# iacopo97/Multimodal-SAM-Adapter

Measured on AMD Instinct MI355X. Metric: images/sec encoder fwd @1024x1024 RGB+LiDAR ViT-L, higher is better.
Workload: dtype split-operand MFMA: fp16 hi + e5m2 cross terms (h8c / h8 planes, ViT / interaction / up-conv GEMMs) fp16 hi/lo pairs x3 (TwinConvNeXt: f3 planes) and bf16 hi/lo x3 (neck, head); attention blocks with the rel-pos terms fused: every contraction on one fp16 MFMA (q, k, v, P rounded to fp16) in the bloc

## Files before the change

include/mmsa.h:

```cpp
#ifndef MMSA_H
#define MMSA_H
#include <stddef.h>
#include <stdint.h>
#ifdef __cplusplus
extern "C" {
#endif

#ifdef MMSA_BUILDING_LIBRARY
typedef hipStream_t mmsa_stream_t;
#else
typedef void* mmsa_stream_t;
#endif

#include "mmsa_version.h"
int mmsa_version(void);
const char* mmsa_last_error(void);

int mmsa_debug_poison_lds(unsigned pattern, mmsa_stream_t stream);
int mmsa_event_create(void** ev);
int mmsa_event_record(void* ev, mmsa_stream_t stream);
int mmsa_event_elapsed_ms(void* start, void* stop, float* ms);
int mmsa_event_destroy(void* ev);

enum { MMSA_ACT_NONE = 0, MMSA_ACT_GELU = 1, MMSA_ACT_RELU = 2, MMSA_ACT_RELU6 = 3, MMSA_ACT_HSWISH = 4, MMSA_ACT_SIGMOID = 5 };

enum { MMSA_DT_F32 = 0, MMSA_DT_F16 = 1, MMSA_DT_F64 = 2 };

enum { MMSA_FMT_B3 = 0, MMSA_FMT_H8 = 1, MMSA_FMT_H8C = 2, MMSA_FMT_F3 = 3, MMSA_FMT_W8 = 4  };

int mmsa_ms_deform_attn_forward(const void* value, const int64_t* spatial_shapes, const int64_t* level_start_index,
                                const void* sampling_loc, const void* attn_weight, void* out, int batch,
                                int spatial_size, int num_heads, int channels, int num_levels, int num_query,
                                int num_point, int im2col_step, int dtype, mmsa_stream_t stream);

int mmsa_ms_deform_attn_backward(const void* value, const int64_t* spatial_shapes, const int64_t* level_start_index,
                                 const void* sampling_loc, const void* attn_weight, const void* grad_output,
                                 void* grad_value, void* grad_sampling_loc, void* grad_attn_weight, int batch,
                                 int spatial_size, int num_heads, int channels, int num_levels, int num_query,
                                 int num_point, int im2col_step, int dtype, mmsa_stream_t stream);

int mmsa_msda_fused(const float* value, const int64_t* spatial_shapes, const int64_t* level_start_index,
                    const float* raw, long ldraw, const float* ref_points, float* out, long ldo,
                    uint16_t* out_planes, long ldop , int out_fmt , int batch,
                    int spatial_size, int num_heads, int channels, int num_levels, int num_query, int num_point,
                    float* clamp_max , mmsa_stream_t stream);

int mmsa_msda_fused_planes(const uint16_t* value_planes, long ldvp, int lo_bytes, const int64_t* spatial_shapes, const int64_t* level_start_index,
                           const float* raw, long ldraw, const float* ref_points, float* out, long ldo,
                           uint16_t* out_planes, long ldop, int out_fmt, int batch,
                           int spatial_size, int num_heads, int channels, int num_levels, int num_query, int num_point,
                           float* clamp_max, mmsa_stream_t stream);

int mmsa_rowstats_finalize(const float* rowstats, int rows, int strips, int D, float eps, float* mean_rstd, mmsa_stream_t stream);

int mmsa_zero_bytes(void* p, size_t bytes, mmsa_stream_t stream);
int mmsa_gemm_split3(const float* A, const uint16_t* Ap, long lda, long strideA,
                     const uint16_t* Wp, long strideW,
                     const float* bias, long strideBias, const float* colscale, const float* resid, long ldr,
                     long strideR, int resid_mod, float beta, float* C, long ldc, long strideC,
                     uint16_t* Cp, long ldcp, long strideCp, int M, int N, int K,
                     int batch, int act, float alpha, int out_mode, int ps_H, int ps_W, int ps_C, int fmt, int cp_fmt,
// ... 122 lines not shown
```

include/mmsa_version.h:

```cpp
#ifndef MMSA_VERSION_H
#define MMSA_VERSION_H
#define MMSA_ABI_VERSION 106
#endif
```

multimodal-sam-adapter_amd/csrc/attention.hip:

```cpp
#include "common.h"

typedef __attribute__((ext_vector_type(4))) short s16x4;
#define LDS_AS __attribute__((address_space(3)))

struct AttnArgs {
  const float* qkv; long ldq;
  const float* qkv_bias;
  const unsigned short* qp;
  const unsigned short* bp;
  unsigned short* op;
  int ofmt;
  int vf;
  const float* rp;
  const unsigned short* relg;
  float* out; long ldo;
  int B, H, W, heads, D;
  int ws;
  int nWw;
  int Nk;
  int KH, KW;
  int KHs, KWs;
  unsigned magicKW;
  float scale;
  float* guard;
};

template <int HD, bool PL, bool FB, bool REL = false, int VF = 0>
__global__ __launch_bounds__(256, (FB && HD <= 64) ? 2 : 1) void attn_kernel(AttnArgs a) {
  static_assert(VF == 0 || PL, "the fp16 paths read planes");
  static_assert(VF != 2 || REL, "the all-fp16 form exists for the fused rel-pos kernel");
  constexpr int NCH = HD / 8;
  constexpr int KS = HD / 32;
  constexpr int DT = HD / 16;
  constexpr int VSTR = 2 * HD + 32;
  constexpr int KPL = NCH * 64 * 16;
  constexpr int VPL = 64 * VSTR;
  extern __shared__ __attribute__((aligned(16))) unsigned char smem[];
  unsigned char* Khi = smem;
  unsigned char* Klo = Khi + KPL;
  unsigned char* Vhi = Klo + KPL;
  unsigned char* Vlo = Vhi + VPL;
  float* bh = reinterpret_cast<float*>(Vlo + VPL);
  float* bw = bh + 128 * a.KHs;

  const int tid = threadIdx.x, lane = tid & 63, wave = tid >> 6;
  const int l15 = lane & 15, G = lane >> 4;
  const unsigned wg_ = mmsa_xcd_order(mmsa_block_lin(), mmsa_block_count());
  const int bx_ = (int)(wg_ % gridDim.x);
  const int head = (int)((wg_ / gridDim.x) % gridDim.y), b = (int)(wg_ / (gridDim.x * gridDim.y));
  const int T = a.H * a.W;
  const int nqb = (a.Nk + 127) / 128;
  const int grp = bx_ / nqb;
  const int q0 = (bx_ % nqb) * 128;
  const int wi = a.ws ? grp / a.nWw : 0, wj = a.ws ? grp % a.nWw : 0;

  auto token_of = [&](int j) -> int {
    if (j >= a.Nk) return -2;
    if (a.ws == 0) return j;
    const int r = j / a.ws, c = j - r * a.ws;
    const int hh = wi * a.ws + r, ww = wj * a.ws + c;
    return (hh < a.H && ww < a.W) ? hh * a.W + ww : -1;
  };
// ... 21 lines not shown
      for (int u = 0; u < 4; ++u) {
        const int i = i0 + 256 * u;
        if (i < total4) {
          const int ql = i / nf4, c4 = i - ql * nf4;
          float* d = bh + ql * a.KHs + 4 * c4;
          d[0] = v[u].x; d[1] = v[u].y; d[2] = v[u].z; d[3] = v[u].w;
        }
      }
    }
  } else {
    const int ncol = a.KH + a.KW;
    const float* rpb = a.rp + ((long)b * a.heads + head) * T * ncol;
    for (int i = tid; i < 128 * ncol; i += 256) {
      const int ql = i / ncol, cidx = i - ql * ncol;
      const int tq = token_of(q0 + ql);
      const float v = tq >= 0 ? rpb[(long)tq * ncol + cidx] : 0.f;
      if (cidx < a.KH) bh[ql * a.KHs + cidx] = v;
      else bw[ql * a.KWs + (cidx - a.KH)] = v;
    }
  }

  bf16x8 qh[2][KS], ql_[2][KS];
  int tq_sub[2];
#pragma unroll
  for (int sub = 0; sub < 2; ++sub) {
    const int jq = q0 + wave * 32 + sub * 16 + l15;
    const int tq = token_of(jq);
    tq_sub[sub] = tq;
    const long qrow = (long)(tq >= 0 ? tq : 0) * a.ldq;
    const float* qp = qkv_b + qrow;
#pragma unroll
    for (int ks = 0; ks < KS; ++ks) {
      if constexpr (PL) {
        const unsigned short* qq = pq_b + qrow + ilv(colq + ks * 32 + 8 * G);
        qh[sub][ks] = *reinterpret_cast<const bf16x8*>(qq);
        if constexpr (VF != 2) ql_[sub][ks] = *reinterpret_cast<const bf16x8*>(qq + 32);
        continue;
      }
      float4 v0 = *reinterpret_cast<const float4*>(qp + ks * 32 + 8 * G);
      float4 v1 = *reinterpret_cast<const float4*>(qp + ks * 32 + 8 * G + 4);
      v0.x *= a.scale; v0.y *= a.scale; v0.z *= a.scale; v0.w *= a.scale;
      v1.x *= a.scale; v1.y *= a.scale; v1.z *= a.scale; v1.w *= a.scale;
      uint2 h0, l0, h1, l1;
      f3_split4(v0, h0, l0);
      f3_split4(v1, h1, l1);
      uint4 hh4 = make_uint4(h0.x, h0.y, h1.x, h1.y), ll4 = make_uint4(l0.x, l0.y, l1.x, l1.y);
      qh[sub][ks] = __builtin_bit_cast(bf16x8, hh4);
      ql_[sub][ks] = __builtin_bit_cast(bf16x8, ll4);
    }
  }

  float bwr[2][4][4];
  if constexpr (REL) {
    float* bwt = reinterpret_cast<float*>(smem);
    int qc[2][2];
#pragma unroll
    for (int sub = 0; sub < 2; ++sub) {
      const int tok = min(q0 + wave * 32 + sub * 16 + l15, a.Nk - 1);
      qc[sub][0] = tok / a.W;
      qc[sub][1] = tok - qc[sub][0] * a.W;
    }
#pragma unroll
    for (int ax = 0; ax < 2; ++ax) {
      const int Kx = ax ? a.KW : a.KH;
      float* tab = ax ? bwt : bh;
      const int tstr = ax ? a.KWs : a.KHs;
#pragma unroll 2
// ... 38 lines not shown
  } else if constexpr (FB) {
    const float* rpb = a.rp + ((long)b * a.heads + head) * T * (a.KH + a.KW) + a.KH;
#pragma unroll
    for (int sub = 0; sub < 2; ++sub) {
      const int tq = tq_sub[sub];
#pragma unroll
      for (int t = 0; t < 4; ++t) {
        float4 v = make_float4(0.f, 0.f, 0.f, 0.f);
        if (tq >= 0) v = *reinterpret_cast<const float4*>(rpb + (long)tq * (a.KH + a.KW) + 16 * t + 4 * G);
        bwr[sub][t][0] = v.x * 1.4426950408889634f;
        bwr[sub][t][1] = v.y * 1.4426950408889634f;
        bwr[sub][t][2] = v.z * 1.4426950408889634f;
        bwr[sub][t][3] = v.w * 1.4426950408889634f;
      }
    }
  }

  constexpr int NF4 = HD / 16;
  constexpr int NU = HD / 32;
  const int skey = (tid & 7) + 8 * (tid >> 5), squart = (tid >> 3) & 3;
  float4 rk[NF4], rv[NF4];
  uint4 rkh[NU], rkl[NU], rvh[NU], rvl[NU];
  unsigned kv_keep = 0xffffffffu;
  auto and4 = [](uint4 v, unsigned m) { return make_uint4(v.x & m, v.y & m, v.z & m, v.w & m); };
#define LOAD_KV(kb_)                                                                         \
  do {                                                                                       \
    const int tk_ = token_of((kb_) * 64 + skey);                                             \
    if constexpr (PL) {                                                                      \
                                                  \
      const unsigned short* rowp_ = tk_ >= 0 ? pq_b + (long)tk_ * a.ldq : a.bp;                                                \
      const unsigned keep_ = tk_ == -2 ? 0u : 0xffffffffu;                                                                     \
      _Pragma("unroll") for (int i = 0; i < NU; ++i) {                                       \
        const int c = squart * (HD / 4) + 8 * i;                                             \
        const unsigned short* kr_ = rowp_ + ilv(colk + c);                                   \
        const unsigned short* vr_ = rowp_ + ilv(colv + c);                                   \
        rkh[i] = *reinterpret_cast<const uint4*>(kr_);                                       \
        if constexpr (VF != 2) rkl[i] = *reinterpret_cast<const uint4*>(kr_ + 32);           \
        rvh[i] = *reinterpret_cast<const uint4*>(vr_);                                       \
        if constexpr (VF == 0) rvl[i] = *reinterpret_cast<const uint4*>(vr_ + 32);           \
      }                                                                                      \
      kv_keep = keep_;                                                                       \
    } else {                                                                                 \
      _Pragma("unroll") for (int i = 0; i < NF4; ++i) {                                      \
        const int c = squart * (HD / 4) + 4 * i;                                             \
        if (tk_ >= 0) {                                                                      \
          const float* p = qkv_b + (long)tk_ * a.ldq + c;                                    \
          rk[i] = *reinterpret_cast<const float4*>(p + a.D);                                 \
          rv[i] = *reinterpret_cast<const float4*>(p + 2 * a.D);                             \
        } else if (tk_ == -1) {                                                              \
          rk[i] = *reinterpret_cast<const float4*>(kbias + c);                               \
          rv[i] = *reinterpret_cast<const float4*>(vbias + c);                               \
        } else {                                                                             \
          rk[i] = make_float4(0.f, 0.f, 0.f, 0.f);                                           \
          rv[i] = rk[i];                                                                     \
        }                                                                                    \
      }                                                                                      \
    }                                                                                        \
  } while (0)
#define STORE_KV(Kh_, Kl_, Vh_, Vl_)                                                                           \
  do {                                                                                       \
    if constexpr (PL) {                                                                      \
      _Pragma("unroll") for (int i = 0; i < NU; ++i) {                                       \
        const int c = squart * (HD / 4) + 8 * i;                                             \
        const int ko = (c >> 3) * (64 * 16) + skey * 16;                                     \
        *reinterpret_cast<uint4*>((Kh_) + ko) = and4(rkh[i], kv_keep);                         \
        if constexpr (VF != 2) *reinterpret_cast<uint4*>((Kl_) + ko) = and4(rkl[i], kv_keep);  \
        const int vo = skey * VSTR + c * 2;                                                  \
        *reinterpret_cast<uint4*>((Vh_) + vo) = and4(rvh[i], kv_keep);                         \
// ... 187 lines not shown
  }

  if (a.guard) {
    const float gv = wave_max(amax) * 0.6931471805599453f;
    if (lane == 0 && gv > *reinterpret_cast<volatile float*>(a.guard)) atomicMax(reinterpret_cast<unsigned*>(a.guard), __float_as_uint(gv));
  }
#pragma unroll
  for (int sub = 0; sub < 2; ++sub) {
    float l = l_run[sub];
    l += __shfl_xor(l, 16, 64);
    l += __shfl_xor(l, 32, 64);
    const float inv = 1.0f / l;
    const int tq = tq_sub[sub];
    if constexpr (PL) {
      const long orow = (long)b * T + (tq >= 0 ? tq : 0);
#pragma unroll
      for (int d = 0; d < DT; ++d)
        store_planes8_pair_any<16>(a.op, a.ldo, orow, MMSA_PAD64(a.D), head * HD + 16 * d + 8 * (G >> 1),
                                   make_float4(o[sub][d][0] * inv, o[sub][d][1] * inv, o[sub][d][2] * inv, o[sub][d][3] * inv), a.ofmt, G & 1, tq >= 0);
    } else if (tq >= 0) {
      const long oo = ((long)b * T + tq) * a.ldo + head * HD + 4 * G;
#pragma unroll
      for (int d = 0; d < DT; ++d)
        *reinterpret_cast<float4*>(a.out + oo + 16 * d) = make_float4(o[sub][d][0] * inv, o[sub][d][1] * inv, o[sub][d][2] * inv, o[sub][d][3] * inv);
    }
  }
}

static int attention_launch(AttnArgs a, int B, int H, int W, int heads, int head_dim, int window_size, float scale,
                            bool planes, hipStream_t stream) {
  MMSA_CHECK_ARG(B > 0 && H > 0 && W > 0 && heads > 0 && window_size >= 0, "attention: bad shape");
  MMSA_CHECK_ARG(head_dim == 64 || head_dim == 32 || head_dim == 96, "attention: head_dim %d not supported (32, 64 or 96; other widths are zero-padded per head by the caller, e.g. ViT-H's 80 -> 96)", head_dim);
  const int D = heads * head_dim;
  MMSA_CHECK_ARG(a.ldq >= (planes ? 6L : 3L) * D && (a.ldq & 7) == 0 && a.ldo >= (planes ? (a.ofmt == MMSA_FMT_H8C ? 3L * MMSA_PAD64(D) : 2L * D) : 1L * D) && (a.ldo & 3) == 0,
                 "attention: bad leading dimensions");
  a.B = B; a.H = H; a.W = W; a.heads = heads; a.D = D; a.ws = window_size; a.scale = scale;
  int ngroups;
  if (window_size > 0) {
    a.nWw = cdiv(W, window_size);
    ngroups = cdiv(H, window_size) * a.nWw;
    a.Nk = window_size * window_size;
    a.KH = a.KW = window_size;
  } else {
    a.nWw = 1;
    ngroups = 1;
    a.Nk = H * W;
    a.KH = H;
    a.KW = W;
  }
  a.KHs = a.KH | 1;
  a.KWs = a.KW | 1;
  a.magicKW = (unsigned)(((1u << 24) + a.KW - 1) / a.KW);
  for (int j = 0; j < a.Nk; ++j) {
    if ((int)(((unsigned long long)(unsigned)j * a.magicKW) >> 24) != j / a.KW || (unsigned long long)j * a.magicKW >= (1ull << 32)) {
      mmsa_set_error("attention: key grid too large for the in-kernel index arithmetic (Nk=%d KW=%d)", a.Nk, a.KW);
      return MMSA_ERR_ARG;
    }
  }
  const int VSTR = 2 * head_dim + 32;
  const bool fb = window_size == 0 && W == 64 && (H % 4) == 0;
  const size_t smem = 2 * (head_dim / 8) * 64 * 16 + 2 * 64 * VSTR + (size_t)128 * (a.KHs + (fb ? 0 : a.KWs)) * sizeof(float);
  MMSA_CHECK_ARG(smem <= 160 * 1024, "attention: bias tables do not fit LDS (KH=%d KW=%d)", a.KH, a.KW);
  dim3 grid(ngroups * cdiv(a.Nk, 128), heads, B);
#define ATTN_LAUNCH(HD_, PL_, FB_)                                                                                         \
  do {                                                                                                                     \
    if (smem > 64 * 1024) (void)hipFuncSetAttribute((const void*)attn_kernel<HD_, PL_, FB_>, hipFuncAttributeMaxDynamicSharedMemorySize, (int)smem); \
    hipLaunchKernelGGL((attn_kernel<HD_, PL_, FB_>), grid, dim3(256), smem, stream, a);                                    \
  } while (0)
#define ATTN_LAUNCH_VF(HD_, FB_)                                                                                           \
  do {                                                                                                                     \
    if (smem > 64 * 1024) (void)hipFuncSetAttribute((const void*)attn_kernel<HD_, true, FB_, false, 1>, hipFuncAttributeMaxDynamicSharedMemorySize, (int)smem); \
    hipLaunchKernelGGL((attn_kernel<HD_, true, FB_, false, 1>), grid, dim3(256), smem, stream, a);                      \
  } while (0)
  MMSA_CHECK_ARG(a.vf == 0 || (planes && a.vf == (a.relg ? 2 : 1)), "attention: v_fmt %d (0 = bf16 hi/lo planes; 1 = h8 planes for the v columns, the entry with a rel-pos prepass; 2 = h8 planes throughout, the fused rel-pos entry)", a.vf);
  if (head_dim == 64) {
    if (planes && a.relg) {
      MMSA_CHECK_ARG(fb && H <= 64 && 128 * a.KWs * (int)sizeof(float) <= 2 * 8 * 64 * 16 + 2 * 64 * VSTR, "attention: the fused rel-pos path needs a W = 64, H <= 64 global grid");
      if (a.vf) hipLaunchKernelGGL((attn_kernel<64, true, true, true, 2>), grid, dim3(256), smem, stream, a);
      else hipLaunchKernelGGL((attn_kernel<64, true, true, true>), grid, dim3(256), smem, stream, a);
    } else if (planes && a.vf) { if (fb) ATTN_LAUNCH_VF(64, true); else ATTN_LAUNCH_VF(64, false); }
    else if (planes) { if (fb) ATTN_LAUNCH(64, true, true); else ATTN_LAUNCH(64, true, false); }
    else { if (fb) ATTN_LAUNCH(64, false, true); else ATTN_LAUNCH(64, false, false); }
  } else if (head_dim == 96) {
    if (planes && a.vf) { if (fb) ATTN_LAUNCH_VF(96, true); else ATTN_LAUNCH_VF(96, false); }
    else if (planes) { if (fb) ATTN_LAUNCH(96, true, true); else ATTN_LAUNCH(96, true, false); }
    else { if (fb) ATTN_LAUNCH(96, false, true); else ATTN_LAUNCH(96, false, false); }
  } else {
    if (planes && a.vf) { if (fb) ATTN_LAUNCH_VF(32, true); else ATTN_LAUNCH_VF(32, false); }
    else if (planes) { if (fb) ATTN_LAUNCH(32, true, true); else ATTN_LAUNCH(32, true, false); }
    else { if (fb) ATTN_LAUNCH(32, false, true); else ATTN_LAUNCH(32, false, false); }
  }
#undef ATTN_LAUNCH_VF
#undef ATTN_LAUNCH
  MMSA_CHECK_LAUNCH("attention");
  return MMSA_OK;
}

extern "C" int mmsa_attention(const float* qkv, long ldq, const float* qkv_bias, const float* rp, float* out, long ldo,
                              int B, int H, int W, int heads, int head_dim, int window_size, float scale,
                              hipStream_t stream) {
  MMSA_CHECK_ARG(qkv && qkv_bias && rp && out, "attention: null pointer");
  MMSA_CHECK_ARG(((((uintptr_t)qkv) | ((uintptr_t)out) | ((uintptr_t)qkv_bias)) & 15) == 0, "attention: pointers must be 16-byte aligned");
  AttnArgs a = {};
  a.qkv = qkv; a.ldq = ldq; a.qkv_bias = qkv_bias; a.rp = rp; a.out = out; a.ldo = ldo;
  return attention_launch(a, B, H, W, heads, head_dim, window_size, scale, false, stream);
}

extern "C" int mmsa_attention_planes(const unsigned short* qkv_p, long ldq, const unsigned short* bias_p, const float* rp,
                                     unsigned short* out_p, long ldo, int B, int H, int W,
                                     int heads, int head_dim, int window_size, float scale, int out_fmt, int v_fmt, float* max_abs_logit,
                                     hipStream_t stream) {
// ... 120 lines not shown
```

multimodal-sam-adapter_amd/csrc/common.h:

```cpp
#pragma once
#include <hip/hip_runtime.h>
#include <stdint.h>
#include <stdio.h>
#include <stdarg.h>

#define MMSA_OK 0
#define MMSA_ERR_ARG (-1)
#define MMSA_ERR_LAUNCH (-2)

#define MMSA_BUILDING_LIBRARY 1
#include "../../include/mmsa.h"
void mmsa_set_error(const char* fmt, ...);

#ifdef MMSA_DEBUG_KNOBS
#include <stdlib.h>
static inline int mmsa_knob_env(const char* name, int dflt) { const char* v = getenv(name); return v ? atoi(v) : dflt; }
#define MMSA_KNOB(name_, dflt_) mmsa_knob_env(name_, dflt_)
#else
#define MMSA_KNOB(name_, dflt_) (dflt_)
#endif

#define MMSA_CHECK_ARG(cond, ...)            \
  do {                                       \
    if (!(cond)) {                           \
// ... 104 lines not shown
__device__ __forceinline__ void f3_split2(float a, float b, unsigned& hi, unsigned& lo) {
  a = __builtin_amdgcn_fmed3f(a, -MMSA_F3_MAX, MMSA_F3_MAX);
  b = __builtin_amdgcn_fmed3f(b, -MMSA_F3_MAX, MMSA_F3_MAX);
  split2_f16(a, b, hi, lo);
}
__device__ __forceinline__ void f3_split4(const float4 v, uint2& hi, uint2& lo) {
  f3_split2(v.x, v.y, hi.x, lo.x);
  f3_split2(v.z, v.w, hi.y, lo.y);
}
__device__ __forceinline__ void split4_fmt(const float4 v, uint2& hi, uint2& lo, int fmt) {
  if (fmt == MMSA_FMT_F3) f3_split4(v, hi, lo);
  else split4(v, hi, lo);
}

template <bool UPPER, bool COMP = false>
__device__ __forceinline__ void h8_split2(float a, float b, unsigned& hi, unsigned& lo8, unsigned& qh8) {
  a = __builtin_amdgcn_fmed3f(a, -MMSA_H8_MAX, MMSA_H8_MAX);
  b = __builtin_amdgcn_fmed3f(b, -MMSA_H8_MAX, MMSA_H8_MAX);
  const mmsa_f32x2 v = {a, b};
  const mmsa_h2 h = __builtin_convertvector(v, mmsa_h2);
  const mmsa_f32x2 hf = __builtin_convertvector(h, mmsa_f32x2);
  constexpr float ls_ = COMP ? MMSA_H8_LO_SCALE * MMSA_H8C_LO_COMP : MMSA_H8_LO_SCALE;
  const mmsa_f32x2 l = (v - hf) * ls_;
  hi = __builtin_bit_cast(unsigned, h);
  lo8 = (unsigned)__builtin_amdgcn_cvt_pk_bf8_f32(l.x, l.y, (int)lo8, UPPER);
  qh8 = (unsigned)__builtin_amdgcn_cvt_pk_bf8_f32(hf.x, hf.y, (int)qh8, UPPER);
}
template <bool COMP = false>
__device__ __forceinline__ void h8_split4(const float4 v, uint2& hi, unsigned& lo8, unsigned& qh8) {
  lo8 = 0u; qh8 = 0u;
  h8_split2<false, COMP>(v.x, v.y, hi.x, lo8, qh8);
  h8_split2<true, COMP>(v.z, v.w, hi.y, lo8, qh8);
}
__host__ __device__ __forceinline__ int h8_lo_off(int c) { return ((c >> 5) << 7) + 64 + (((c & 31) >> 3) << 4) + (c & 7); }

__device__ __forceinline__ void store_planes4(unsigned short* row, int c, const float4 v, int fmt) {
  if (fmt == MMSA_FMT_H8) {
    uint2 hi; unsigned lo8, qh8;
    h8_split4(v, hi, lo8, qh8);
    *reinterpret_cast<uint2*>(row + ilv(c)) = hi;
    unsigned char* rb = reinterpret_cast<unsigned char*>(row) + h8_lo_off(c);
    *reinterpret_cast<unsigned*>(rb) = lo8;
    *reinterpret_cast<unsigned*>(rb + 8) = qh8;
  } else {
    uint2 hh, ll;
    split4_fmt(v, hh, ll, fmt);
    *reinterpret_cast<uint2*>(row + ilv(c)) = hh;
    *reinterpret_cast<uint2*>(row + ilv(c) + 32) = ll;
  }
}

template <int XOR>
__device__ __forceinline__ void store_planes8_pair(unsigned short* row, int c8, const float4 v, int fmt, bool odd, bool do_store) {
  uint2 mine_hi, mine_x;
  if (fmt == MMSA_FMT_H8) h8_split4(v, mine_hi, mine_x.x, mine_x.y);
  else split4_fmt(v, mine_hi, mine_x, fmt);
  const uint2 snd = odd ? mine_hi : mine_x;
  uint2 rcv;
  rcv.x = __shfl_xor(snd.x, XOR, 64);
  rcv.y = __shfl_xor(snd.y, XOR, 64);
  uint4 pk;
  if (!odd) pk = make_uint4(mine_hi.x, mine_hi.y, rcv.x, rcv.y);
  else if (fmt == MMSA_FMT_H8) pk = make_uint4(rcv.x, mine_x.x, rcv.y, mine_x.y);
  else pk = make_uint4(rcv.x, rcv.y, mine_x.x, mine_x.y);
  const int off = odd ? (fmt == MMSA_FMT_H8 ? h8_lo_off(c8) >> 1 : ilv(c8) + 32) : ilv(c8);
  if (do_store) *reinterpret_cast<uint4*>(row + off) = pk;
// ... 170 lines not shown
```

multimodal-sam-adapter_amd/csrc/gemm_epilogue_regs.inc:

```
#ifndef MMSA_EPI_REGS
#define MMSA_EPI_REGS 1
#endif
#ifndef MMSA_EPI_REGS_FP32
#define MMSA_EPI_REGS_FP32 0
#endif
#ifndef MMSA_EPI_ROWS
#define MMSA_EPI_ROWS 1
#endif
#ifndef MMSA_EPI_NOSTORE
#define MMSA_EPI_NOSTORE 0
#endif
#if MMSA_EPI_NOSTORE
#define EPI_ST16(ptr_, val_) { const uint4 v__ = __builtin_bit_cast(uint4, val_); asm volatile("" :: "v"(v__.x), "v"(v__.y), "v"(v__.z), "v"(v__.w), "v"(ptr_)); }
#else
#define EPI_ST16(ptr_, val_) { *reinterpret_cast<uint4*>(ptr_) = __builtin_bit_cast(uint4, val_); }
#endif
#ifndef EPI_STAMP
#define EPI_STAMP(i_)
#define EPI_STAMP_WAIT()
#define EPI_STAMP_DEFAULTED_ 1
#endif
      bool regs_done = false;
      if constexpr (MMSA_EPI_REGS && EPI_UNROLL && !GEN && (ACT == ACT_NONE || ACT == ACT_GELU)) {
        const bool interior_ = m0 + V2_BM <= a.M && n0 + a.bn <= a.N;
        const bool al16_ = ((((uintptr_t)bias) | ((uintptr_t)colscale) | ((uintptr_t)resid) | ((uintptr_t)C) | ((uintptr_t)Cp) | ((uintptr_t)a.rn_cs)) & 15) == 0 &&
                           ((a.ldc | a.ldr) & 3) == 0 && (a.ldcp & 7) == 0 && (a.strideBias & 3) == 0;
        if (interior_ && al16_ && V2_DBG(a) == 0 && !cp_split && (ni4 || (C && !Cp && !a.rs_out && !a.rn_mr))) {
          auto swap16_ = [](unsigned& x_, unsigned& y_) {
            const auto r_ = __builtin_amdgcn_permlane16_swap(x_, y_, false, false);
            x_ = r_[0]; y_ = r_[1];
          };
          auto epi_regs_ = [&](auto c_C, auto c_R, auto c_CPF, auto c_RS, auto c_RN, auto c_CS) {
// ... 13 lines not shown
              }
              if constexpr (kRN) sn_[ni] = *reinterpret_cast<const float4*>(a.rn_cs + (long)bz * a.strideBias + ci);
            }
            float2 mr_[4];
            if constexpr (kRN) {
#pragma unroll
              for (int mi = 0; mi < 4; ++mi) mr_[mi] = *reinterpret_cast<const float2*>(a.rn_mr + 2 * ((long)bz * a.M + row0 + 16 * mi));
            }
#ifndef MMSA_EPI_PREFETCH_ALL
#define MMSA_EPI_PREFETCH_ALL 0
#endif
            float4 rra[4][4];
            const float* rbase = nullptr;
            if constexpr (kR) {
              rbase = resid + (long)row0 * a.ldr + col0;
#pragma unroll
              for (int mi = 0; mi < (MMSA_EPI_PREFETCH_ALL ? 4 : 1); ++mi)
#pragma unroll
                for (int ni = 0; ni < 4; ++ni) rra[mi][ni] = *reinterpret_cast<const float4*>(rbase + (long)mi * 16 * a.ldr + ni * 16);
            }
            EPI_STAMP(1) EPI_STAMP_WAIT() EPI_STAMP(2)
            float* cbase = nullptr;
            if constexpr (kC) cbase = C + (long)row0 * a.ldc + col0;
            const int hcol = 16 * (g & 1) + 8 * (g >> 1);
            const int schunk = 16 * (2 * (g & 1) + (g >> 1));
            unsigned short* prow = nullptr;
            unsigned char* plo = nullptr;
            long pstep = 0;
            if constexpr (kCPF == MMSA_FMT_H8C) {
              unsigned short* pb = Cp + (long)(row0 >> 1) * a.ldcp;
              prow = pb + (row0 & 1) * cp_kpad + nb_ + hcol;
              plo = reinterpret_cast<unsigned char*>(pb + 2 * cp_kpad) + (row0 & 1) * 64 + ((nb_ >> 6) << 7) + schunk;
              pstep = 8 * a.ldcp;
            } else if constexpr (kCPF >= 0) {
              prow = Cp + (long)row0 * a.ldcp + ((nb_ >> 5) << 6) + hcol;
              pstep = 16 * a.ldcp;
            }
            unsigned long long cwm_ = 0ull;
            constexpr bool kWatch = MMSA_CLAMP_WATCH && MMSA_CW_REGS && (kCPF == MMSA_FMT_H8C || kCPF == MMSA_FMT_H8 || kCPF == MMSA_FMT_F3);
            constexpr float kLimit = (kCPF == MMSA_FMT_F3) ? MMSA_F3_MAX : MMSA_H8_MAX;
            float* rsb = nullptr;
            if constexpr (kRS) rsb = a.rs_out + (((long)bz * a.M + row0) * a.rs_strips + (nb_ >> 6)) * 2;
#pragma unroll
            for (int mi = 0; mi < 4; ++mi) {
              if constexpr (kR && !MMSA_EPI_PREFETCH_ALL) {
                if (mi < 3) {
#pragma unroll
                  for (int ni = 0; ni < 4; ++ni) rra[mi + 1][ni] = *reinterpret_cast<const float4*>(rbase + (long)(mi + 1) * 16 * a.ldr + ni * 16);
                }
              }
              float s1 = 0.f, s2 = 0.f;
              uint2 H[4], Lp[4];
              unsigned L8[4], Q8[4];
#pragma unroll
              for (int ni = 0; ni < 4; ++ni) {
                float4 o;
                if constexpr (kRN) {
                  const float mu = mr_[mi].x, rs = mr_[mi].y;
                  o = make_float4(fmaf(rs, fmaf(-mu, sn_[ni].x, acc[ni][mi][0]), bn_[ni].x), fmaf(rs, fmaf(-mu, sn_[ni].y, acc[ni][mi][1]), bn_[ni].y),
                                  fmaf(rs, fmaf(-mu, sn_[ni].z, acc[ni][mi][2]), bn_[ni].z), fmaf(rs, fmaf(-mu, sn_[ni].w, acc[ni][mi][3]), bn_[ni].w));
                } else {
                  o = make_float4(acc[ni][mi][0] + bn_[ni].x, acc[ni][mi][1] + bn_[ni].y, acc[ni][mi][2] + bn_[ni].z, acc[ni][mi][3] + bn_[ni].w);
                }
                acc[ni][mi] = (f32x4){0.f, 0.f, 0.f, 0.f};
                if constexpr (ACT == ACT_GELU) o = gelu4(o);
                if constexpr (kCS) { o.x *= cn_[ni].x; o.y *= cn_[ni].y; o.z *= cn_[ni].z; o.w *= cn_[ni].w; }
                if constexpr (kR) { o.x += a.beta * rra[mi][ni].x; o.y += a.beta * rra[mi][ni].y; o.z += a.beta * rra[mi][ni].z; o.w += a.beta * rra[mi][ni].w; }
                if constexpr (kC) EPI_ST16(cbase + (long)mi * 16 * a.ldc + ni * 16, o)
                if constexpr (kRS) {
                  s1 += (o.x + o.y) + (o.z + o.w);
                  s2 += fmaf(o.x, o.x, o.y * o.y) + fmaf(o.z, o.z, o.w * o.w);
                }
                if constexpr (kWatch) cwm_ |= __builtin_amdgcn_ballot_w64(fmaxf(fmaxf(fabsf(o.x), fabsf(o.y)), fmaxf(fabsf(o.z), fabsf(o.w))) > kLimit);
                if constexpr (kCPF == MMSA_FMT_H8C) h8_split4<true>(o, H[ni], L8[ni], Q8[ni]);
                else if constexpr (kCPF == MMSA_FMT_H8) h8_split4<false>(o, H[ni], L8[ni], Q8[ni]);
                else if constexpr (kCPF == MMSA_FMT_F3) f3_split4(o, H[ni], Lp[ni]);
                else if constexpr (kCPF == MMSA_FMT_B3) split4(o, H[ni], Lp[ni]);
              }
              if constexpr (kCPF >= 0) {
                unsigned short* pr = prow + (long)mi * pstep;
#pragma unroll
                for (int p = 0; p < 2; ++p) {
                  swap16_(H[2 * p].x, H[2 * p + 1].x);
                  swap16_(H[2 * p].y, H[2 * p + 1].y);
                  const uint4 hv = make_uint4(H[2 * p].x, H[2 * p].y, H[2 * p + 1].x, H[2 * p + 1].y);
                  if constexpr (kCPF == MMSA_FMT_H8C) {
                    EPI_ST16(pr + 32 * p, hv)
                  } else {
                    EPI_ST16(pr + 64 * p, hv)
                    if constexpr (kCPF == MMSA_FMT_H8) {
                      swap16_(L8[2 * p], L8[2 * p + 1]);
                      swap16_(Q8[2 * p], Q8[2 * p + 1]);
                      EPI_ST16(reinterpret_cast<unsigned char*>(pr + 64 * p - hcol) + 64 + schunk, make_uint4(L8[2 * p], L8[2 * p + 1], Q8[2 * p], Q8[2 * p + 1]))
                    } else {
                      swap16_(Lp[2 * p].x, Lp[2 * p + 1].x);
                      swap16_(Lp[2 * p].y, Lp[2 * p + 1].y);
                      EPI_ST16(pr + 64 * p + 32, make_uint4(Lp[2 * p].x, Lp[2 * p].y, Lp[2 * p + 1].x, Lp[2 * p + 1].y))
                    }
                  }
                }
                if constexpr (kCPF == MMSA_FMT_H8C) {
                  swap16_(L8[0], L8[1]);
                  swap16_(L8[2], L8[3]);
                  EPI_ST16(plo + (long)mi * pstep * 2, make_uint4(L8[0], L8[1], L8[2], L8[3]))
                }
              }
              if constexpr (kRS) {
                {
                  const auto r1 = __builtin_amdgcn_permlane32_swap(__float_as_uint(s1), __float_as_uint(s1), false, false);
                  const auto r2 = __builtin_amdgcn_permlane32_swap(__float_as_uint(s2), __float_as_uint(s2), false, false);
                  s1 = __uint_as_float(r1[0]) + __uint_as_float(r1[1]);
                  s2 = __uint_as_float(r2[0]) + __uint_as_float(r2[1]);
                }
                {
                  const auto r1 = __builtin_amdgcn_permlane16_swap(__float_as_uint(s1), __float_as_uint(s1), false, false);
                  const auto r2 = __builtin_amdgcn_permlane16_swap(__float_as_uint(s2), __float_as_uint(s2), false, false);
                  s1 = __uint_as_float(r1[0]) + __uint_as_float(r1[1]);
                  s2 = __uint_as_float(r2[0]) + __uint_as_float(r2[1]);
                }
// ... 40 lines not shown
#pragma unroll
                  for (int i = 0; i < 4; ++i) rq[(mi + 1) & 1][i] = *reinterpret_cast<const float4*>(rb_ + (long)(16 * (mi + 1) + 4 * i) * a.ldr);
                }
              }
#pragma unroll
              for (int ni = 0; ni < 4; ++ni) {
                *reinterpret_cast<f32x4*>(stg_ + l15 * 68 + ni * 16 + 4 * g) = acc[ni][mi];
                acc[ni][mi] = (f32x4){0.f, 0.f, 0.f, 0.f};
              }
#pragma unroll
              for (int i = 0; i < 4; ++i) {
                const float4 t = *reinterpret_cast<const float4*>(stg_ + (rl + 4 * i) * 68 + cl4);
                float4 o;
                if constexpr (kRN) {
                  const float mu = mr4[mi][i].x, rs = mr4[mi][i].y;
                  o = make_float4(fmaf(rs, fmaf(-mu, sn4.x, t.x), bv4.x), fmaf(rs, fmaf(-mu, sn4.y, t.y), bv4.y), fmaf(rs, fmaf(-mu, sn4.z, t.z), bv4.z), fmaf(rs, fmaf(-mu, sn4.w, t.w), bv4.w));
                } else {
                  o = make_float4(t.x + bv4.x, t.y + bv4.y, t.z + bv4.z, t.w + bv4.w);
                }
                if constexpr (kCS) { o.x *= cv4.x; o.y *= cv4.y; o.z *= cv4.z; o.w *= cv4.w; }
                if constexpr (kR) { const float4 r_ = rq[mi & 1][i]; o.x += a.beta * r_.x; o.y += a.beta * r_.y; o.z += a.beta * r_.z; o.w += a.beta * r_.w; }
                EPI_ST16(cb_ + (long)(16 * mi + 4 * i) * a.ldc, o)
              }
              EPI_STAMP(3 + mi)
            }
          };
          const int cpf_ = Cp ? cp_base : -1;
          const bool rn_ = a.rn_mr != nullptr, rso_ = a.rs_out != nullptr;
          const bool scaled_ = colscale != nullptr || a.alpha != 1.0f;
#define EPI_REGS_RUN1(C_, R_, F_, S_, N_, CS_)                                                                                        \
  { epi_regs_(std::integral_constant<bool, C_>{}, std::integral_constant<bool, R_>{}, std::integral_constant<int, F_>{},               \
              std::integral_constant<bool, S_>{}, std::integral_constant<bool, N_>{}, std::integral_constant<bool, CS_>{}); regs_done = true; }
#define EPI_REGS_RUN(C_, R_, F_, S_, N_) { if (!scaled_) EPI_REGS_RUN1(C_, R_, F_, S_, N_, false) }
          if (!C && !resid && !rso_) {
            if (cpf_ == MMSA_FMT_H8C) { if (rn_) EPI_REGS_RUN(false, false, MMSA_FMT_H8C, false, true) else EPI_REGS_RUN(false, false, MMSA_FMT_H8C, false, false) }
            else if (cpf_ == MMSA_FMT_H8) { if (rn_) EPI_REGS_RUN(false, false, MMSA_FMT_H8, false, true) else EPI_REGS_RUN(false, false, MMSA_FMT_H8, false, false) }
            else if (cpf_ == MMSA_FMT_F3 && !rn_) EPI_REGS_RUN(false, false, MMSA_FMT_F3, false, false)
            else if (cpf_ == MMSA_FMT_B3 && !rn_) EPI_REGS_RUN(false, false, MMSA_FMT_B3, false, false)
          } else if (C && cpf_ < 0 && !rso_ && MMSA_EPI_ROWS) {
            if constexpr (ACT == ACT_NONE) {
              if (scaled_) {
                if (!rn_) { if (resid) epi_rows_(std::true_type{}, std::false_type{}, std::true_type{}); else epi_rows_(std::false_type{}, std::false_type{}, std::true_type{}); regs_done = true; }
              } else if (resid) { if (!rn_) { epi_rows_(std::true_type{}, std::false_type{}, std::false_type{}); regs_done = true; } }
              else if (rn_) { epi_rows_(std::false_type{}, std::true_type{}, std::false_type{}); regs_done = true; }
              else { epi_rows_(std::false_type{}, std::false_type{}, std::false_type{}); regs_done = true; }
            }
          } else if (C && !rn_) {
            if constexpr (ACT == ACT_NONE) {
              if (resid && rso_ && cpf_ == MMSA_FMT_H8C) { if (scaled_) EPI_REGS_RUN1(true, true, MMSA_FMT_H8C, true, false, true) else EPI_REGS_RUN1(true, true, MMSA_FMT_H8C, true, false, false) }
              else if (resid && rso_ && cpf_ == MMSA_FMT_F3) EPI_REGS_RUN(true, true, MMSA_FMT_F3, true, false)
              else if (MMSA_EPI_REGS_FP32 && resid && !rso_ && cpf_ < 0) EPI_REGS_RUN(true, true, -1, false, false)
              else if (MMSA_EPI_REGS_FP32 && !resid && !rso_ && cpf_ < 0) EPI_REGS_RUN(true, false, -1, false, false)
            }
          }
#undef EPI_REGS_RUN
#undef EPI_REGS_RUN1
#undef EPI_ST16
        }
      }
```

multimodal-sam-adapter_amd/csrc/gemm_h8c.hip:

```cpp
#include "common.h"
#include "gemm_h8c_shared.h"

#define HC_H_UNIT 49152
#define HC_L_UNIT 24576
#define HC_LDS_H(i_) ((i_) * HC_H_UNIT)
#define HC_LDS_L(i_) (2 * HC_H_UNIT + (i_) * (HC_L_UNIT + 16384))
#define HC_LDS_TOTAL (2 * HC_H_UNIT + 2 * HC_L_UNIT + 16384)

#ifdef HC_EPI_STAMP
__device__ unsigned long long g_hc_estamps[8 * 16];
extern "C" int mmsa_debug_epi_stamps(unsigned long long* host_out) { return (int)hipMemcpyFromSymbol(host_out, HIP_SYMBOL(g_hc_estamps), sizeof(g_hc_estamps)); }
#define EPI_STAMP(i_) { if (estamp_on_) { __builtin_amdgcn_sched_barrier(0); et_[i_] = __builtin_readcyclecounter(); __builtin_amdgcn_sched_barrier(0); } }
#define EPI_STAMP_WAIT() { if (estamp_on_) asm volatile("s_waitcnt vmcnt(0)" ::: "memory"); }
#else
#define EPI_STAMP(i_)
#define EPI_STAMP_WAIT()
#endif
template <bool GEN, int ACT>
__global__ __launch_bounds__(512, 1) void gemm_h8c_kernel(GemmV2Args a) {
  constexpr bool PP = true;
  constexpr bool EPI_UNROLL = ACT >= 0;
  constexpr int V2_BM = 256;
  constexpr int V2_NST = 3;
  extern __shared__ __attribute__((aligned(16))) unsigned char smem[];
  const int tid = threadIdx.x, lane = tid & 63;
  const int wave = __builtin_amdgcn_readfirstlane(tid >> 6);
  const int wm = wave >> 1, wn = wave & 1, grp = wave >> 2;
  const int l15 = lane & 15, g = lane >> 4;
  const int K = a.K;
  const int np = K >> 6;
  const bool ni4 = true;
  const int swid = 64;
  const int G = gridDim.x;
  int rb = blockIdx.x;
  V2_XCD_REMAP(rb, G)
  const int my_tiles = (a.ntiles - rb + G - 1) / G;
  if (my_tiles <= 0) return;
  V2_SLACK_STAGGER(a, rb, G)
  const int total = my_tiles * np;

  H8C_DMA_LANE();
  const int lds_ha = wave * 32 * 128, lds_hw = 32768 + wave * 16 * 128;
  const int lds_la = wave * 2048, lds_lw = 16384 + wave * 1024;
  const unsigned ldaB = (unsigned)(a.lda * 2), ldwB = (unsigned)(a.ldw * 2);
  const unsigned K2 = (unsigned)K * 2u, K4 = (unsigned)K * 4u;
  H8C_A_LANE_HI();
  const unsigned LW_E = (unsigned)(drow >> 1) * ldwB + (unsigned)(drow & 1) * K2 + dpiece, LW_O = LW_E ^ 64u;
  H8C_A_LANE_LO();
  const unsigned LLW = (unsigned)drow * ldwB + K4 + lq;

  const unsigned char *hA, *hW, *lA, *lW;
  int h_m0 = 0, h_n0 = 0, l_m0 = 0, l_n0 = 0;
// ... 106 lines not shown
    H8C_SB();                                                                                                         \
     \
     \
    if (FAST_) { ++lp_j; ++lp_p; ++hp_j; ++hp_p; } else { if (do_l) HC_L_ADVANCE() if (do_h) HC_H_ADVANCE() }          \
    H8C_SB();                                                                                                         \
    if (FAST_) H8C_WAIT(9); else if (tail || last) H8C_WAIT(0); else if (!skipw) H8C_WAIT(9);                         \
    H8C_BAR()                                                                                                         \
    if (!(FAST_)) nowait = 0;                                                                                         \
    ++j;                                                                                                              \
  }

  for (int tdone = 0; tdone < my_tiles; ++tdone) {
    if (grp) H8C_BAR()
    bool interior;
    { int bz_, m0_, n0_; H8C_TILE(tile, 256, bz_, m0_, n0_) interior = m0_ + 256 <= a.M && n0_ + 128 <= a.N; }
    int p = 0;
    HC_PAIR(0)
    ++p;
    if (interior) {
#pragma unroll 1
      for (; p < np - 2; ++p) HC_PAIR(1)
      if (hp_p == np) { hp_p = 0; hp_tile += G; if (hp_j < total) HC_SET_H(hp_tile) }
    }
#pragma unroll 1
    for (; p < np; ++p) HC_PAIR(0)
    if (!grp) H8C_BAR()
    if (V2_DBG(a) == 2) H8C_NO_EPILOGUE() else {
#ifdef HC_EPI_STAMP
      unsigned long long et_[9] = {0, 0, 0, 0, 0, 0, 0, 0, 0};
      const bool estamp_on_ = blockIdx.x == 0 && tdone == 1;
#endif
      EPI_STAMP(0)
#define EPI_STAGING_BASE (smem + (((j - 1) & 1) ? 2 * HC_H_UNIT + HC_L_UNIT : 2 * HC_H_UNIT))
#include "gemm_v2_epilogue.inc"
      EPI_STAMP(7)
#ifdef HC_EPI_STAMP
      asm volatile("s_waitcnt lgkmcnt(0)" ::: "memory");
      H8C_BAR()
      EPI_STAMP(8)
      if (estamp_on_ && (threadIdx.x & 63) == 0) {
#pragma unroll
        for (int q_ = 0; q_ < 9; ++q_) g_hc_estamps[wave * 16 + q_] = et_[q_];
      }
#endif
    }
    asm volatile("s_waitcnt lgkmcnt(0)" ::: "memory");
    H8C_BAR()
    tile += G;
  }
}

int mmsa_gemm_h8c_dispatch(const GemmV2Args& a, int grid, bool gen, int act, hipStream_t stream) {
  static MmsaPerDevice per_dev_ = {};
  (void)mmsa_per_device(per_dev_, [] {
#define HC_ATTR(GEN_, ACT_) (void)hipFuncSetAttribute((const void*)gemm_h8c_kernel<GEN_, ACT_>, hipFuncAttributeMaxDynamicSharedMemorySize, HC_LDS_TOTAL);
    V2_EPI_TABLE(HC_ATTR)
#undef HC_ATTR
  });
#define HC_LAUNCH(GEN_, ACT_) if (v2_epi_serves(gen, act, GEN_, ACT_)) hipLaunchKernelGGL((gemm_h8c_kernel<GEN_, ACT_>), dim3(grid), dim3(512), HC_LDS_TOTAL, stream, a);
  V2_EPI_TABLE(HC_LAUNCH)
#undef HC_LAUNCH
  MMSA_CHECK_LAUNCH("gemm_split3(h8c)");
  return MMSA_OK;
}
```

multimodal-sam-adapter_amd/csrc/gemm_h8c_w8.hip:

```cpp
#include "gemm_h8c_shared.h"

typedef __attribute__((ext_vector_type(2))) _Float16 hw_h2;

#define HW_H_UNIT 40960
#define HW_L_UNIT 32768
#define HW_LDS_H(i_) ((i_) * HW_H_UNIT)
#define HW_LDS_L(i_) (2 * HW_H_UNIT + (i_) * (HW_L_UNIT + 16384))
#define HW_LDS_TOTAL (2 * HW_H_UNIT + 2 * HW_L_UNIT + 16384)

__device__ __forceinline__ uint2 w8_cvt4(unsigned c, float s) {
  const hw_h2 lo = __builtin_amdgcn_cvt_scalef32_pk_f16_fp8(c, s, false);
  const hw_h2 hi = __builtin_amdgcn_cvt_scalef32_pk_f16_fp8(c, s, true);
  return make_uint2(__builtin_bit_cast(unsigned, lo), __builtin_bit_cast(unsigned, hi));
}

template <bool GEN, int ACT>
__global__ __launch_bounds__(512, 1) void gemm_h8c_w8_kernel(GemmV2Args a) {
  constexpr bool PP = true;
  constexpr bool EPI_UNROLL = ACT >= 0;
  constexpr int V2_BM = 256;
  constexpr int V2_NST = 3;
  extern __shared__ __attribute__((aligned(16))) unsigned char smem[];
  const int tid = threadIdx.x, lane = tid & 63;
  const int wave = __builtin_amdgcn_readfirstlane(tid >> 6);
  const int wm = wave >> 1, wn = wave & 1, grp = wave >> 2;
  const int l15 = lane & 15, g = lane >> 4;
  const int K = a.K;
  const int np = K >> 6;
  const bool ni4 = true;
  const int swid = 64;
  const int G = gridDim.x;
  int rb = blockIdx.x;
  V2_XCD_REMAP(rb, G)
  const int my_tiles = (a.ntiles - rb + G - 1) / G;
  if (my_tiles <= 0) return;
  V2_SLACK_STAGGER(a, rb, G)
  const int total = my_tiles * np;
  const int nsteps = np >> 1, total_s = my_tiles * nsteps;

  H8C_DMA_LANE();
  const int lds_ha = wave * 32 * 128, lds_hw = 32768 + wave * 1024;
  const int lds_la = wave * 2048;
  const unsigned ldaB = (unsigned)(a.lda * 2);
  const unsigned ldwB = (unsigned)(a.ldw * 2);
  const unsigned K2 = (unsigned)K * 2u, K4 = (unsigned)K * 4u;
  H8C_A_LANE_HI();
  const int wcol = lane >> 2;
  const unsigned wpiece = (unsigned)(((lane & 3) ^ ((lane >> 4) & 3)) * 16);
  const unsigned LW = (unsigned)wcol * ldwB + wpiece;
  H8C_A_LANE_LO();
// ... 143 lines not shown
    H8C_SB();                                                                                                         \
    if (tail || last) H8C_WAIT(0); else if ((FAST_) || !skipw) { if (ODD_) H8C_WAIT(5); else H8C_WAIT(9); }          \
    H8C_BAR()                                                                                                         \
    if (!(FAST_)) nowait = 0;                                                                                         \
    ++j;                                                                                                              \
  }

  for (int tdone = 0; tdone < my_tiles; ++tdone) {
    if (grp) H8C_BAR()
    bool interior;
    { int bz_, m0_, n0_; H8C_TILE(tile, 256, bz_, m0_, n0_) interior = m0_ + 256 <= a.M && n0_ + 128 <= a.N; }
    HW_SCALES(tile)
    int p = 0;
    HW_PAIR(0, 0)
    ++p;
    HW_PAIR(0, 1)
    ++p;
    if (interior) {
#pragma unroll 1
      for (; p < np - 2; p += 2) { HW_PAIR(1, 0) HW_PAIR(1, 1) }
      if (hp_p == np) { hp_p = 0; hp_tile += G; if (hp_j < total) HW_SET_H(hp_tile) }
      if (lp_p == nsteps) { lp_p = 0; lp_tile += G; if (lp_j < total_s) HW_SET_L(lp_tile) }
    }
#pragma unroll 1
    for (; p < np; ) {
      HW_PAIR(0, 0)
      ++p;
      HW_PAIR(0, 1)
      ++p;
    }
    if (!grp) H8C_BAR()
    if (V2_DBG(a) == 2) H8C_NO_EPILOGUE() else {
#define EPI_STAGING_BASE (smem + ((((j - 1) >> 1) & 1) ? HW_LDS_L(1) - 16384 : HW_LDS_L(0)))
#include "gemm_v2_epilogue.inc"
    }
    asm volatile("s_waitcnt lgkmcnt(0)" ::: "memory");
    H8C_BAR()
    tile += G;
  }
}

int mmsa_gemm_h8c_w8_dispatch(const GemmV2Args& a, int grid, bool gen, int act, hipStream_t stream) {
  static MmsaPerDevice per_dev_ = {};
  (void)mmsa_per_device(per_dev_, [] {
#define HW_ATTR(GEN_, ACT_) (void)hipFuncSetAttribute((const void*)gemm_h8c_w8_kernel<GEN_, ACT_>, hipFuncAttributeMaxDynamicSharedMemorySize, HW_LDS_TOTAL);
    V2_EPI_TABLE(HW_ATTR)
#undef HW_ATTR
  });
#define HW_LAUNCH(GEN_, ACT_) if (v2_epi_serves(gen, act, GEN_, ACT_)) hipLaunchKernelGGL((gemm_h8c_w8_kernel<GEN_, ACT_>), dim3(grid), dim3(512), HW_LDS_TOTAL, stream, a);
  V2_EPI_TABLE(HW_LAUNCH)
#undef HW_LAUNCH
  MMSA_CHECK_LAUNCH("gemm_split3(h8c x w8)");
  return MMSA_OK;
}
```

multimodal-sam-adapter_amd/csrc/gemm_split3.hip:

```cpp
#include "common.h"

struct GemmArgs {
  const float* A; const unsigned short* Ap; long lda; long strideA;
  const unsigned short* Wp; long strideW;
  const float* bias; long strideBias;
  const float* colscale;
  const float* resid; long ldr; long strideR; int resid_mod; float beta;
  float* C; long ldc; long strideC;
  unsigned short* Cp; long ldcp; long strideCp;
  int M, N, K;
  int act; float alpha;
  int out_mode; int ps_H, ps_W, ps_C;
  int cp_fmt;
  float* clamp_max;
};

#define BM 128
#define BN 128
#define BK 32
#define PLANE_BYTES (4 * 128 * 16)
#define STAGE_BYTES (4 * PLANE_BYTES)

template <bool AP, bool GEN, bool F16 = false>
__global__ __launch_bounds__(256) void gemm_split3_kernel(GemmArgs a) {
// ... 253 lines not shown
#pragma unroll
  for (int j = 0; j < 8; ++j) acc[j] = wave_sum(acc[j]);
  if (lane < 8 && n0 + lane < a.N) {
    const int n = n0 + lane;
    float v = acc[0];
#pragma unroll
    for (int j = 1; j < 8; ++j) v = lane == j ? acc[j] : v;
    if (a.bias) v += a.bias[(long)bz * a.strideBias + n];
    v = apply_act(v, a.act) * (a.colscale ? a.colscale[(long)bz * a.strideBias + n] * a.alpha : a.alpha);
    if (a.resid) v += a.beta * a.resid[(long)bz * a.strideR + (long)m * a.ldr + n];
    a.C[(long)bz * a.strideC + (long)m * a.ldc + n] = v;
  }
}


extern "C" int mmsa_gemm_split3(const float* A, const unsigned short* Ap, long lda, long strideA,
                                const unsigned short* Wp, long strideW,
                                const float* bias, long strideBias, const float* colscale,
                                const float* resid, long ldr, long strideR, int resid_mod, float beta,
                                float* C, long ldc, long strideC,
                                unsigned short* Cp, long ldcp, long strideCp,
                                int M, int N, int K, int batch, int act, float alpha,
                                int out_mode, int ps_H, int ps_W, int ps_C, int fmt, int cp_fmt, int max_grid,
                                float* rowstats_out, const float* rownorm_mean_rstd, const float* rownorm_colsum, int flavour,
                                float* clamp_max, hipStream_t stream) {
  const bool ap = Ap != nullptr;
  float* const rs_out = rowstats_out;
  const float* const rn_mr = rownorm_mean_rstd;
  const float* const rn_cs = rownorm_colsum;
  MMSA_CHECK_ARG(!rn_mr == !rn_cs, "gemm_split3: mean/rstd rows and column sums go together");
  MMSA_CHECK_ARG(!(rs_out && rn_mr), "gemm_split3: a GEMM either writes row statistics or normalises by them");
  const bool extras = rs_out || rn_mr;
  MMSA_CHECK_ARG(!extras || (ap && M >= 128), "gemm_split3: row statistics / row normalisation need activation planes and M >= 128");
  MMSA_CHECK_ARG(fmt >= MMSA_FMT_B3 && fmt <= MMSA_FMT_W8 && cp_fmt >= 0 && MMSA_CP_BASE(cp_fmt) >= MMSA_FMT_B3 && MMSA_CP_BASE(cp_fmt) <= MMSA_FMT_F3, "gemm_split3: bad plane format %d / %d", fmt, cp_fmt);
  MMSA_CHECK_ARG(MMSA_CP_SPLIT(cp_fmt) == 0 || (out_mode == 0 && MMSA_CP_SPLIT(cp_fmt) < N && MMSA_CP_BASE(cp_fmt) != MMSA_FMT_H8C), "gemm_split3: the output-format split %d needs a plain [M, N] bf16 hi/lo planes output with N=%d beyond it", MMSA_CP_SPLIT(cp_fmt), N);
  MMSA_CHECK_ARG(fmt == MMSA_FMT_B3 || fmt == MMSA_FMT_F3 || (ap && K % 64 == 0), "gemm_split3: h8 / h8c operands need A planes and K %% 64 == 0 (K=%d)", K);
  MMSA_CHECK_ARG(fmt != MMSA_FMT_F3 || ap || !Cp, "gemm_split3: f3 weights with an fp32 A write fp32 outputs only");
  MMSA_CHECK_ARG(fmt != MMSA_FMT_W8 || (K % 128 == 0 && batch == 1), "gemm_split3: W8 weights need h8c A planes, K %% 128 == 0 and one batch (K=%d, batch=%d)", K, batch);
  const bool h8c = fmt == MMSA_FMT_H8C || fmt == MMSA_FMT_W8, cp_h8c = MMSA_CP_BASE(cp_fmt) == MMSA_FMT_H8C;
  MMSA_CHECK_ARG((A || Ap) && Wp && (C || Cp), "gemm_split3: null pointer");
  MMSA_CHECK_ARG(!(A && Ap), "gemm_split3: pass either fp32 A or A planes, not both");
  MMSA_CHECK_ARG(M > 0 && N > 0 && K > 0 && batch > 0, "gemm_split3: bad shape M=%d N=%d K=%d batch=%d", M, N, K, batch);
  MMSA_CHECK_ARG(K % BK == 0, "gemm_split3: K=%d must be a multiple of %d (producers pad)", K, BK);
  if (ap) {
    MMSA_CHECK_ARG((lda & 63) == 0 && (strideA & 63) == 0 && (((uintptr_t)Ap) & 127) == 0,
                   "gemm_split3: A planes must be 128-byte aligned with lda%%64==0 (lda=%ld)", lda);
    MMSA_CHECK_ARG(lda >= (h8c ? 3L : 2L) * K, "gemm_split3: planes lda=%ld < %d*K=%d (h8c: lda is the row-PAIR stride)", lda, h8c ? 3 : 2, K);
  } else {
    MMSA_CHECK_ARG((lda & 3) == 0 && (strideA & 3) == 0 && (((uintptr_t)A) & 15) == 0, "gemm_split3: A must be 16-byte aligned with lda%%4==0 (lda=%ld)", lda);
  }
  MMSA_CHECK_ARG(lda >= K, "gemm_split3: lda=%ld < K=%d", lda, K);
  MMSA_CHECK_ARG((((uintptr_t)Wp) & 127) == 0 && (strideW & 63) == 0, "gemm_split3: weight planes must be 128-byte aligned");
  MMSA_CHECK_ARG((!C || (((uintptr_t)C) & 15) == 0) && (!resid || (((uintptr_t)resid) & 15) == 0), "gemm_split3: C/resid must be 16-byte aligned");
  MMSA_CHECK_ARG(!Cp || ((((uintptr_t)Cp) & 127) == 0 && (ldcp & 63) == 0 && (strideCp & 63) == 0), "gemm_split3: output planes must be 128-byte aligned, ldcp%%64==0");
  MMSA_CHECK_ARG(act >= ACT_NONE && act <= ACT_SIGMOID, "gemm_split3: bad act %d", act);
  if (out_mode == 1) {
    MMSA_CHECK_ARG(ps_H > 0 && ps_W > 0 && ps_C > 0 && N == 4 * ps_C && M % (ps_H * ps_W) == 0 && (ps_C & 3) == 0,
                   "gemm_split3: pixel-shuffle store needs N==4*C, M%%(H*W)==0");
    MMSA_CHECK_ARG((!C || ldc >= ps_C) && (!Cp || ldcp >= (cp_h8c ? 3L * MMSA_PAD64(ps_C) : 2L * ps_C)), "gemm_split3: ldc < C");
  } else {
    MMSA_CHECK_ARG(out_mode == 0, "gemm_split3: bad out_mode %d", out_mode);
    MMSA_CHECK_ARG((!C || ldc >= N) && (!Cp || ldcp >= (cp_h8c ? 3L * MMSA_PAD64(N) : 2L * ((N + 31) / 32 * 32))), "gemm_split3: ldc=%ld < N=%d", ldc, N);
  }
  GemmArgs a;
  a.A = A; a.Ap = Ap; a.lda = lda; a.strideA = strideA;
  a.Wp = Wp; a.strideW = strideW;
  a.bias = bias; a.strideBias = strideBias; a.colscale = colscale;
  a.resid = resid; a.ldr = ldr; a.strideR = strideR; a.resid_mod = resid_mod; a.beta = beta;
  a.C = C; a.ldc = C ? ldc : 0; a.strideC = strideC;
  a.Cp = Cp; a.ldcp = Cp ? ldcp : 0; a.strideCp = strideCp;
  a.M = M; a.N = N; a.K = K; a.act = act; a.alpha = alpha;
  a.out_mode = out_mode; a.ps_H = ps_H; a.ps_W = ps_W; a.ps_C = ps_C; a.cp_fmt = cp_fmt;
  a.clamp_max = clamp_max;
  const bool force_v1 = MMSA_KNOB("MMSA_GEMM_V1", 0) != 0;
  const bool narrow = false;
  const bool no_tiny = MMSA_KNOB("MMSA_GEMM_NO_TINY", 0) != 0;
  if (!ap && !Cp && out_mode == 0 && resid_mod <= 0 && (N <= 64 || K <= 64) && M <= 16384 && !no_tiny && !extras && fmt == MMSA_FMT_B3) {
    const int ncg = cdiv(N, 8);
    hipLaunchKernelGGL(gemm_tiny_kernel, dim3(cdiv((long)M * ncg, 4), batch), dim3(256), 0, stream, a, ncg);
    MMSA_CHECK_LAUNCH("gemm_split3(tiny)");
    return MMSA_OK;
  }
  if (ap && (fmt != MMSA_FMT_B3 || (M >= 128 && !force_v1 && !narrow))) {
    return mmsa_gemm_v2_launch(Ap, lda, strideA, Wp, strideW, bias, strideBias, colscale, resid, ldr, strideR,
                               resid_mod, beta, C, ldc, strideC, Cp, ldcp, strideCp, M, N, K, batch, act, alpha,
                               out_mode, ps_H, ps_W, ps_C, fmt, cp_fmt, max_grid, stream, rs_out, rn_mr, rn_cs, flavour, clamp_max);
  }
  MMSA_CHECK_ARG(!extras, "gemm_split3: this shape is not routed to the LDS-DMA kernel, which alone writes row statistics / normalises rows");
  MMSA_CHECK_ARG(!cp_h8c, "gemm_split3: h8c output planes are written by the LDS-DMA kernel only (activation planes in, M >= 128)");
  dim3 grid(cdiv(N, BN), cdiv(M, BM), batch);
  const bool gen = out_mode != 0 || resid_mod > 0;
  if (ap) {
    if (gen) hipLaunchKernelGGL((gemm_split3_kernel<true, true>), grid, dim3(256), 2 * STAGE_BYTES, stream, a);
    else hipLaunchKernelGGL((gemm_split3_kernel<true, false>), grid, dim3(256), 2 * STAGE_BYTES, stream, a);
  } else if (fmt == MMSA_FMT_F3) {
// ... 55 lines not shown
```

multimodal-sam-adapter_amd/csrc/gemm_v2.hip:

```cpp
#include "common.h"
#include "gemm_v2_shared.h"
template <bool GEN, int ACT, bool PP, int NW, int FMT>
__global__ __launch_bounds__(NW * 64, NW == 4 ? 2 : 1) void gemm_v2_kernel(GemmV2Args a) {
  static_assert(NW == 8 || (NW == 4 && !PP), "4-wave workgroups run the in-phase main loop");
  static_assert(FMT == MMSA_FMT_B3 || (PP && NW == 8), "the h8 and f3 operand formats run on the ping-pong kernel");
  constexpr bool EPI_UNROLL = ACT >= 0;
  constexpr int V2_BM = NW * 32;
  constexpr int V2_A_BYTES = V2_BM * 128;
  constexpr int V2_STAGE = V2_A_BYTES + V2_W_BYTES;
  constexpr int V2_NST = NW == 8 ? 3 : 2;
  constexpr int WROWS = V2_BN / NW;
  constexpr int NDMA = 4 + WROWS / 8;
  extern __shared__ __attribute__((aligned(16))) unsigned char smem[];
  const int tid = threadIdx.x;
  const int lane = tid & 63;
  const int wave = __builtin_amdgcn_readfirstlane(tid >> 6);
  const int wm = wave >> 1, wn = wave & 1;
  const int grp = wave >> 2;
  const int l15 = lane & 15, g = lane >> 4;
  const int K = a.K;
  const int nk = K / V2_BK;

  const int G = gridDim.x;
  int rb = blockIdx.x;
  V2_XCD_REMAP(rb, G)
  const int my_tiles = (a.ntiles - rb + G - 1) / G;
  if (my_tiles <= 0) return;
  V2_SLACK_STAGGER(a, rb, G)
  CLK_SAMPLE(0)
  const int total = my_tiles * nk;

  const int drow = lane >> 3;
  const int dpiece = ((lane & 7) ^ (drow >> 1)) * 8;
  const int lds_a = wave * 32 * 128;
  const int lds_w = wave * WROWS * 128;
  const unsigned char *gA, *gW;
// ... 362 lines not shown
#undef MXPAR
        }
      } else {
#define MXPAR 0
#pragma unroll 1
        for (int kt = 0; kt < kt_a; ++kt) K_STEP_PP()
        if (ni4) {
#pragma unroll 1
          for (int kt = kt_a; kt < kt_b; ++kt) K_STEP_PP_FAST(true)
        } else {
#pragma unroll 1
          for (int kt = kt_a; kt < kt_b; ++kt) K_STEP_PP_FAST(false)
        }
        if (fast_ok) {
          pf_kt = 0;
          pf_tile += G;
          if (pf_j < total) SET_TILE_SRC(pf_tile);
        }
#pragma unroll 1
        for (int kt = kt_b; kt < nk; ++kt) K_STEP_PP()
#undef MXPAR
      }
      if (!grp) __builtin_amdgcn_s_barrier();
    } else {
#define MXPAR 0
#pragma unroll 1
      for (int kt = 0; kt < nk; ++kt) K_STEP()
#undef MXPAR
    }
    const int st_cur = st == 0 ? V2_NST - 1 : st - 1;

    if (V2_DBG(a) == 2 || V2_DBG(a) == 5 || V2_DBG(a) >= 64) { tile += G; continue; }
#define EPI_STAGING_BASE (smem + st_cur * V2_STAGE)
#include "gemm_v2_epilogue.inc"
    if constexpr (PP) {
      asm volatile("s_waitcnt lgkmcnt(0)" ::: "memory");
      __builtin_amdgcn_s_barrier();
    }
    tile += G;
  }
  CLK_SAMPLE(2)
#undef K_STEP
#undef K_STEP_PP
#undef K_STEP_PP_FAST
#undef PP_WAIT
#undef PP_PIECE
#undef MFMA_CHUNK
#undef MFMA_FP8_ALL
}

int mmsa_gemm_h8c_dispatch(const GemmV2Args& a, int grid, bool gen, int act, hipStream_t stream);
int mmsa_gemm_h8c_w8_dispatch(const GemmV2Args& a, int grid, bool gen, int act, hipStream_t stream);
int mmsa_gemm_stream_try(const unsigned short* Ap, long lda, const unsigned short* Wp, const float* bias, const float* colscale, const float* resid, long ldr, float beta,
                         float* C, long ldc, unsigned short* Cp, long ldcp, int M, int N, int K, int batch, int act, float alpha, int out_mode, int resid_mod,
                         int fmt, int cp_fmt, int max_grid, const float* rs_out, const float* rn_mr, int flavour, float* clamp_max, hipStream_t stream);
int mmsa_gemm_h8c4_dispatch(const GemmV2Args& a, int grid, hipStream_t stream);

int mmsa_gemm_v2_launch(const unsigned short* Ap, long lda, long strideA,
                        const unsigned short* Wp, long strideW,
                        const float* bias, long strideBias, const float* colscale,
                        const float* resid, long ldr, long strideR, int resid_mod, float beta,
                        float* C, long ldc, long strideC,
                        unsigned short* Cp, long ldcp, long strideCp,
                        int M, int N, int K, int batch, int act, float alpha,
                        int out_mode, int ps_H, int ps_W, int ps_C, int fmt, int cp_fmt, int max_grid, hipStream_t stream,
                        float* rs_out, const float* rn_mr, const float* rn_cs, int flavour, float* clamp_max) {
// ... 9 lines not shown
  MMSA_CHECK_ARG(!rn_mr || (rn_cs && !resid && out_mode == 0 && resid_mod <= 0 && (N & 127) == 0 && ((((uintptr_t)bias) | ((uintptr_t)colscale) | ((uintptr_t)rn_cs)) & 15) == 0 && (strideBias & 3) == 0 &&
                            ((Cp && !C && (act == ACT_NONE || act == ACT_GELU || act == ACT_RELU)) ||
                             (C && !Cp && act == ACT_NONE && (M & 255) == 0 && !colscale && alpha == 1.0f && (ldc & 3) == 0 && (((uintptr_t)C) & 15) == 0))),
                 "gemm(v2): the row-normalising epilogue needs N %% 128 == 0 (N=%d), 16-byte aligned column vectors and either a planes-only output or a plain fp32 output with M %% 256 == 0 (M=%d), no activation / scale", N, M);
  a.rs_out = rs_out; a.rs_strips = N >> 6; a.rn_mr = rn_mr; a.rn_cs = rn_cs;
  a.Ap = Ap; a.lda = lda; a.strideA = strideA;
  a.Wp = Wp; a.strideW = strideW;
  const bool w8 = fmt == MMSA_FMT_W8;
  const bool h8c = fmt == MMSA_FMT_H8C || w8;
  MMSA_CHECK_ARG(!w8 || ((K & 127) == 0 && batch == 1), "gemm(v2): W8 weights need K %% 128 == 0 and one batch (K=%d, batch=%d)", K, batch);
  a.ldw = w8 ? K / 2 : h8c ? 3L * K : 2L * K;
  a.bias = bias; a.strideBias = strideBias; a.colscale = colscale;
  a.resid = resid; a.ldr = ldr; a.strideR = strideR; a.resid_mod = resid_mod; a.beta = beta;
  a.C = C; a.ldc = C ? ldc : 0; a.strideC = strideC;
  a.Cp = Cp; a.ldcp = Cp ? ldcp : 0; a.strideCp = strideCp;
  a.M = M; a.N = N; a.K = K; a.act = act; a.alpha = alpha;
  a.out_mode = out_mode; a.ps_H = ps_H; a.ps_W = ps_W; a.ps_C = ps_C;
  auto log2_exact = [](int v) { int s_ = -1; if (v > 0 && (v & (v - 1)) == 0) { s_ = 0; while ((1 << s_) < v) ++s_; } return s_; };
  a.ps_sw = log2_exact(ps_W); a.ps_sh = log2_exact(ps_H);
  a.cp_fmt = cp_fmt;
  const bool h8 = fmt == MMSA_FMT_H8 || h8c;
  MMSA_CHECK_ARG(!h8 || (K & 63) == 0, "gemm(v2): h8 operands need K %% 64 == 0 (K=%d)", K);
  MMSA_CHECK_ARG(flavour == 0 || flavour == 4 || flavour == 8, "gemm(v2): flavour %d (0 = by shape, 4, 8)", flavour);
  static MmsaPerDevice per_dev_ = {};
  const int num_cus = mmsa_per_device(per_dev_, [] {
#define V2_ATTR(GEN_, ACT_)                                                                                                   \
  (void)hipFuncSetAttribute((const void*)gemm_v2_kernel<GEN_, ACT_, false, 8, MMSA_FMT_B3>, hipFuncAttributeMaxDynamicSharedMemorySize, V2_LDS_BYTES(8)); \
  (void)hipFuncSetAttribute((const void*)gemm_v2_kernel<GEN_, ACT_, true, 8, MMSA_FMT_B3>, hipFuncAttributeMaxDynamicSharedMemorySize, V2_LDS_BYTES(8));  \
  (void)hipFuncSetAttribute((const void*)gemm_v2_kernel<GEN_, ACT_, true, 8, MMSA_FMT_H8>, hipFuncAttributeMaxDynamicSharedMemorySize, V2_LDS_BYTES(8));  \
  (void)hipFuncSetAttribute((const void*)gemm_v2_kernel<GEN_, ACT_, true, 8, MMSA_FMT_F3>, hipFuncAttributeMaxDynamicSharedMemorySize, V2_LDS_BYTES(8));  \
  (void)hipFuncSetAttribute((const void*)gemm_v2_kernel<GEN_, ACT_, false, 4, MMSA_FMT_B3>, hipFuncAttributeMaxDynamicSharedMemorySize, V2_LDS_BYTES(4));
    V2_EPI_TABLE(V2_ATTR)
#undef V2_ATTR
  });
  const int cus = (max_grid > 0 && max_grid < num_cus) ? max_grid : num_cus;
  const bool h8c4 = flavour == 4 && h8c && !w8 && out_mode == 0 && resid_mod <= 0 && act == ACT_NONE && M >= 128;
  const int nw = h8c4 ? 4 : (h8 || rs_out || rn_mr || fmt == MMSA_FMT_F3) ? 8 : flavour ? flavour : (K <= MMSA_KNOB("MMSA_GEMM_NW4_MAXK", 256) && max_grid <= 0 ? 4 : 8);
  const int bm = nw * 32, wg_per_cu = nw == 4 ? 2 : 1;
  a.nbm = cdiv(M, bm);
  a.bn = V2_BN;
  a.nbn = cdiv(N, V2_BN);
  a.ntiles = a.nbm * a.nbn * batch;
#ifdef MMSA_DEBUG_KNOBS
  a.debug = MMSA_KNOB("MMSA_GEMM_DEBUG", 0);
#endif
  if (!Cp && out_mode == 0 && resid_mod <= 0 && N >= 96 && N % 96 == 0 && !rs_out && !h8c) {
    const bool no96 = MMSA_KNOB("MMSA_GEMM_NO96", 0) != 0;
    const int nbn96 = cdiv(N, 96);
    const long t96 = (long)a.nbm * nbn96 * batch;
    const int slots = cus * wg_per_cu;
    const double c128 = (double)cdiv(a.ntiles, slots), c96 = 0.75 * (double)cdiv(t96, slots);
    if (!no96 && c96 < c128 - 1e-9) {
      a.bn = 96;
      a.nbn = nbn96;
      a.ntiles = (int)t96;
    }
  }
  const bool rowmajor = MMSA_KNOB("MMSA_GEMM_ROWMAJOR", 0) != 0;
  a.tm = a.tn = 0;
  if (!rowmajor) {
    double best = 0.0;
    for (int tn = 1; tn <= 32; tn <<= 1) {
      const int tm = 32 / tn;
      if (a.nbn % tn != 0 || a.nbm % tm != 0) continue;
      const double cost = (double)(a.nbn / tn) * M + (double)(a.nbm / tm) * N;
      if (a.tm == 0 || cost < best) { best = cost; a.tm = tm; a.tn = tn; }
    }
  }
  const int slots_ = cus * wg_per_cu;
  const int rounds_ = cdiv(a.ntiles, slots_);
  int grid = cdiv(a.ntiles, rounds_);
  a.stagger = 0;
#ifndef MMSA_GEMM_STAGGER
#define MMSA_GEMM_STAGGER 0
#endif
  if (MMSA_GEMM_STAGGER && MMSA_KNOB("MMSA_GEMM_STAGGER", 1) && nw == 8 && rounds_ >= 2 && a.ntiles % slots_ != 0) {
    grid = slots_;
    a.stagger = h8c ? (K >> 6) * 3800 + 16000 : (K >> 5) * (fmt == MMSA_FMT_H8 ? 1700 : 1900) + 16000;
  }
  const bool gen = out_mode != 0 || resid_mod > 0;
  if (w8) return mmsa_gemm_h8c_w8_dispatch(a, grid, gen, act, stream);
  if (h8c4) return mmsa_gemm_h8c4_dispatch(a, grid, stream);
  if (h8c) return mmsa_gemm_h8c_dispatch(a, grid, gen, act, stream);
  const bool pp = MMSA_KNOB("MMSA_GEMM_PP", 1) != 0;
#define V2_LAUNCH(GEN_, ACT_)                                                                                              \
  if (v2_epi_serves(gen, act, GEN_, ACT_)) {                                                                               \
    if (fmt == MMSA_FMT_H8) hipLaunchKernelGGL((gemm_v2_kernel<GEN_, ACT_, true, 8, MMSA_FMT_H8>), dim3(grid), dim3(512), V2_LDS_BYTES(8), stream, a);          \
    else if (fmt == MMSA_FMT_F3) hipLaunchKernelGGL((gemm_v2_kernel<GEN_, ACT_, true, 8, MMSA_FMT_F3>), dim3(grid), dim3(512), V2_LDS_BYTES(8), stream, a);     \
    else if (nw == 4) hipLaunchKernelGGL((gemm_v2_kernel<GEN_, ACT_, false, 4, MMSA_FMT_B3>), dim3(grid), dim3(256), V2_LDS_BYTES(4), stream, a);     \
    else if (pp) hipLaunchKernelGGL((gemm_v2_kernel<GEN_, ACT_, true, 8, MMSA_FMT_B3>), dim3(grid), dim3(512), V2_LDS_BYTES(8), stream, a);     \
    else hipLaunchKernelGGL((gemm_v2_kernel<GEN_, ACT_, false, 8, MMSA_FMT_B3>), dim3(grid), dim3(512), V2_LDS_BYTES(8), stream, a);            \
  }
  V2_EPI_TABLE(V2_LAUNCH)
#undef V2_LAUNCH
  MMSA_CHECK_LAUNCH("gemm_split3(v2)");
  return MMSA_OK;
}
```

multimodal-sam-adapter_amd/csrc/gemm_v2_epilogue.inc:

```
    {
      int lane_o_ = lane;
      asm volatile("" : "+v"(lane_o_));
      const int lane = lane_o_, l15 = lane_o_ & 15, g = lane_o_ >> 4;
    {
      const int per_b = a.nbm * a.nbn;
      const int bz = tile / per_b;
      const int rt = tile - bz * per_b;
      int tmi, tni;
      V2_TILE_MN(rt, tmi, tni);
      const int m0 = tmi * V2_BM, n0 = tni * a.bn;
      const float* bias = a.bias ? a.bias + (long)bz * a.strideBias : nullptr;
      const float* colscale = a.colscale ? a.colscale + (long)bz * a.strideBias : nullptr;
      const float* resid = a.resid ? a.resid + (long)bz * a.strideR : nullptr;
      float* C = a.C ? a.C + (long)bz * a.strideC : nullptr;
      unsigned short* Cp = a.Cp ? a.Cp + (long)bz * a.strideCp : nullptr;
      const bool vec_ok = ((a.ldc & 3) == 0) && (!resid || (a.ldr & 3) == 0) && ((a.N & 3) == 0) && ((a.ldcp & 3) == 0);
      if constexpr (PP) {
        nowait = 1;
      } else {
        asm volatile("s_waitcnt vmcnt(0)" ::: "memory");
        asm volatile("s_waitcnt lgkmcnt(0)" ::: "memory");
        __builtin_amdgcn_s_barrier();
        nowait = V2_NST - 1;
      }
      float* stg = reinterpret_cast<float*>(EPI_STAGING_BASE) + wave * (16 * 68);
      const int nb_ = n0 + wn * swid;
      const int cp_base = MMSA_CP_BASE(a.cp_fmt);
      const bool cp_split = MMSA_CP_SPLIT(a.cp_fmt) != 0;
      const bool cp_h8c = cp_base == MMSA_FMT_H8C;
      const int cp_kpad = MMSA_PAD64((GEN && a.out_mode == 1) ? a.ps_C : a.N);
#include "gemm_epilogue_regs.inc"
      if (!regs_done) {
      const float cw_lim_ = cp_split ? MMSA_H8_MAX : mmsa_clamp_limit(cp_base);
      auto cp_stage4 = [&](unsigned short* srow_, int c_, const float4 o_, int col_) {
#if MMSA_CW_LEG
        { float m_ = 0.f; clamp_see(m_, o_); clamp_report(a.clamp_max, m_, cw_lim_); }
#endif
        if (cp_h8c) {
          uint2 hi_; unsigned lo8_, qh8_;
          h8_split4<true>(o_, hi_, lo8_, qh8_);
          *reinterpret_cast<uint2*>(srow_ + c_) = hi_;
          *reinterpret_cast<unsigned*>(reinterpret_cast<unsigned char*>(srow_) + 128 + h8c_lo_off(c_)) = lo8_;
        } else {
          store_planes4(srow_, c_, o_, cp_split ? MMSA_CP_AT(a.cp_fmt, col_) : cp_base);
        }
      };
      auto cp_store16 = [&](long drow__, int dcol__, const uint4 pk_) {
        if (cp_h8c) {
          const H8cRow r_ = h8c_row(Cp, a.ldcp, drow__, cp_kpad);
          const int l_ = lane & 15, ch_ = (dcol__ >> 6) << 7;
          if (l_ < 8) *reinterpret_cast<uint4*>(reinterpret_cast<unsigned char*>(r_.hi) + ch_ + 16 * l_) = pk_;
          else if (l_ < 12) *reinterpret_cast<uint4*>(r_.lo + ch_ + 16 * (l_ - 8)) = pk_;
        } else {
          *reinterpret_cast<uint4*>(Cp + drow__ * a.ldcp + ilv(dcol__ & ~63) + 8 * (lane & 15)) = pk_;
        }
      };
      auto cp_store1 = [&](long drow__, int dcol__, float x_) {
#if MMSA_CW_LEG
        clamp_report(a.clamp_max, fabsf(x_), cw_lim_);
#endif
        if (cp_h8c) h8c_store1(h8c_row(Cp, a.ldcp, drow__, cp_kpad), dcol__, x_);
        else store_planes1(Cp + drow__ * a.ldcp, dcol__, x_, MMSA_CP_AT(a.cp_fmt, dcol__));
      };
      const int rl0 = lane >> 4;
      const int cl = (lane & 15) * 4;
      const bool lane_ok = cl < swid;
      const int n = nb_ + (lane_ok ? cl : 0);
      float bv[4], cv[4];
#pragma unroll
      for (int r = 0; r < 4; ++r) {
        int ci = min(n + r, a.N - 1);
        bv[r] = bias ? bias[ci] : 0.f;
        if constexpr (GEN) { if (a.out_mode == 1) ci %= a.ps_C; }
        cv[r] = colscale ? colscale[ci] * a.alpha : a.alpha;
      }
      int ij_n = 0, dcol_n = n;
      if constexpr (GEN) { if (a.out_mode == 1) { ij_n = n / a.ps_C; dcol_n = n - ij_n * a.ps_C; } }
      auto map_row = [&](int m, int nn, long& drow_, int& dcol, long& rrow) {
        drow_ = m; dcol = nn; rrow = m;
        if constexpr (GEN) {
          if (a.out_mode == 1) {
            int ij = ij_n;
            dcol = dcol_n;
            if (nn != n) { ij = nn / a.ps_C; dcol = nn - ij * a.ps_C; }
            int w_, h_, b_;
            if (a.ps_sw >= 0 && a.ps_sh >= 0) {
              w_ = m & (a.ps_W - 1);
              const int t_ = m >> a.ps_sw;
              h_ = t_ & (a.ps_H - 1);
              b_ = t_ >> a.ps_sh;
            } else {
              w_ = m % a.ps_W;
              const int t_ = m / a.ps_W;
              h_ = t_ % a.ps_H;
// ... 187 lines not shown
              long drow_, rrow; int dcol;
              map_row(m, n, drow_, dcol, rrow);
              if (C) *reinterpret_cast<float4*>(C + drow_ * a.ldc + dcol) = o;
              if (Cp) cp_store16(drow_, dcol, pk);
            }
          }
        } else {
#pragma unroll 1
          for (int e = 0; e < 16; ++e) {
            const int i = e >> 2, r = e & 3;
            const int rl = rl0 + 4 * i;
            const int m = mb + rl;
            if (m >= a.M || n + r >= a.N || !lane_ok) continue;
            float x = stg[rl * 68 + cl + r];
            {
              int ci = n + r;
              const float b_ = bias ? bias[ci] : 0.f;
              if constexpr (GEN) { if (a.out_mode == 1) ci %= a.ps_C; }
              x = apply_act(x + b_, act) * (colscale ? colscale[ci] * a.alpha : a.alpha);
            }
            long drow_, rrow; int dcol;
            map_row(m, n + r, drow_, dcol, rrow);
            if (resid) x += a.beta * resid[rrow * a.ldr + dcol];
            if (C) C[drow_ * a.ldc + dcol] = x;
            if (Cp) cp_store1(drow_, dcol, x);
          }
        }
        }
      }
      }
    }
    }
#undef EPI_STAGING_BASE
#ifdef EPI_STAMP_DEFAULTED_
#undef EPI_STAMP_DEFAULTED_
#undef EPI_STAMP
#undef EPI_STAMP_WAIT
#endif
```

multimodal-sam-adapter_amd/csrc/wattn.hip:

```cpp
#include "common.h"

typedef __attribute__((ext_vector_type(4))) short s16x4;
#define LDS_AS __attribute__((address_space(3)))
#define GLDS16(gptr, lptr)                                                                                  \
  __builtin_amdgcn_global_load_lds((const __attribute__((address_space(1))) void*)(gptr),                   \
                                   (__attribute__((address_space(3))) void*)(lptr), 16, 0, 0)

#define WA_WAVES 13
#ifndef WP_FOLD
#define WP_FOLD 1
#endif
#define WA_NKEY 208
#define WA_NKV 224
#define WA_K_BYTES (2 * WA_NKEY * 128)
#define WA_V_BYTES (WA_NKV * 128)
#define WA_E_BYTES (WA_NKEY * 64)
#define WA_B_BYTES (16 * 128)
#define WA_LDS (WA_K_BYTES + 2 * WA_V_BYTES + WA_E_BYTES + WA_WAVES * WA_B_BYTES)

struct WAttnArgs {
  const unsigned short* qp; long ldq;
  const unsigned short* bp;
  const unsigned short* relp;
  const unsigned short* sel;
  unsigned short* op; long ldo;
  int ofmt;
  int B, H, W, heads, D, ws, nWw;
  float* guard;
  unsigned magic;
  float scale;
#ifdef MMSA_DEBUG_KNOBS
  long long* stamps;
#endif
};
#ifdef MMSA_DEBUG_KNOBS
static long long* g_wattn_stamps = nullptr;
extern "C" int mmsa_debug_wattn_stamps(long long* p) { g_wattn_stamps = p; return MMSA_OK; }
#define WP_STAMP(k_)                                                                                                         \
  do {                                                                                                                       \
    if (a.stamps && blockIdx.x == 0 && (wave == 0 || wave == 6) && lane == 0 && nst_ < 8)                                    \
      a.stamps[((wave ? 1 : 0) * 8 + nst_) * 16 + (k_)] = (long long)__builtin_amdgcn_s_memtime();                           \
  } while (0)
#else
#define WP_STAMP(k_) do { } while (0)
#endif

#define WP_NKV 208
#define WP_V_BYTES (WP_NKV * 128)
#define WP_R_BYTES (2 * 64 * 128)
#define WP_LDS (WA_K_BYTES + 2 * WP_V_BYTES + WA_E_BYTES + WP_R_BYTES + WA_WAVES * WA_B_BYTES)

template <bool VF>
__global__ __launch_bounds__(WA_WAVES * 64) void wattn_persist_kernel(WAttnArgs a, int nWin, int nitems) {
  extern __shared__ __attribute__((aligned(16))) unsigned char smem[];
  unsigned char* Ks = smem;
  unsigned char* Vhi = smem + WA_K_BYTES;
  unsigned char* Vlo = Vhi + WP_V_BYTES;
  unsigned char* Es = Vlo + WP_V_BYTES;
  unsigned char* Rs = Es + WA_E_BYTES;
  const int tid = threadIdx.x, lane = tid & 63;
  const int wave = __builtin_amdgcn_readfirstlane(tid >> 6);
  float* Bw = reinterpret_cast<float*>(Rs + WP_R_BYTES + wave * WA_B_BYTES);
  const int l15 = lane & 15, G = lane >> 4;
  const int T = a.H * a.W, ws = a.ws, Nk = ws * ws;
  const int dr = lane >> 3, slot = lane & 7;

  int wi, wj, head, b;
  const int nWh = nWin / a.nWw, nHB = a.heads * a.B;
  auto decode = [&](int it) {
    const int r = it / nHB;
    const int hb = it - r * nHB;
    head = hb % a.heads;
    b = hb / a.heads;
    const int nI = (nWh - 1) * (a.nWw - 1);
    if (r < nI) {
      wi = r / (a.nWw - 1);
      wj = r - wi * (a.nWw - 1);
    } else if (r - nI < nWh - 1) {
      wi = r - nI;
      wj = a.nWw - 1;
    } else {
      wi = nWh - 1;
      wj = r - nI - (nWh - 1);
    }
  };
  auto token_of = [&](int j) -> int {
    if (j >= Nk) return -2;
    const int r = (int)(__umul24(j, a.magic) >> 16), c = j - __umul24(r, ws);
    const int hh = wi * ws + r, ww = wj * ws + c;
    return (hh < a.H && ww < a.W) ? hh * a.W + ww : -1;
  };
#define WP_ISSUE_K()                                                                                          \
  {                                                                                                           \
    int lo_ = lane;       \
    asm volatile("" : "+v"(lo_));                                                                             \
    const int dr = lo_ >> 3, slot = lo_ & 7;                                                                  \
    const unsigned short* pq_b_ = a.qp + (long)b * T * a.ldq;                                                 \
    const int colk_ = a.D + head * 64;                                                                        \
    _Pragma("unroll") for (int half = 0; half < 2; ++half) {                                                  \
      const int key = 16 * wave + 8 * half + dr;                                                              \
      const int t_ = token_of(key);                                                                           \
      const unsigned short* row = t_ >= 0 ? pq_b_ + (long)t_ * a.ldq : a.bp;                                  \
      const int piece = slot ^ ((key & 15) >> 1);                                                             \
      GLDS16(row + 2 * colk_ + piece * 8, Ks + (16 * wave + 8 * half) * 128);                                 \
      GLDS16(row + 2 * (colk_ + 32) + piece * 8, Ks + (WA_NKEY + 16 * wave + 8 * half) * 128);                \
    }                                                                                                         \
  }
#define WP_ISSUE_V()                                                                                          \
  {                                                                                                           \
    int lo_ = lane;                                                                                           \
    asm volatile("" : "+v"(lo_));                                                                             \
    const int dr = lo_ >> 3, slot = lo_ & 7;                                                                  \
    const unsigned short* pq_b_ = a.qp + (long)b * T * a.ldq;                                                 \
    const int colv_ = 2 * a.D + head * 64;                                                                    \
    _Pragma("unroll") for (int half = 0; half < 2; ++half) {                                                  \
      const int key = 16 * wave + 8 * half + dr;                                                              \
      const int t_ = token_of(key);                                                                           \
      const unsigned short* row = t_ >= 0 ? pq_b_ + (long)t_ * a.ldq : a.bp;                                  \
      const int c = slot ^ (((key >> 1) & 3) << 1);                                                           \
      const unsigned short* vsrc = row + 2 * (colv_ + 32 * (c >> 2)) + (c & 3) * 8;                           \
      GLDS16(vsrc, Vhi + (16 * wave + 8 * half) * 128);                                                       \
      if constexpr (!VF) GLDS16(vsrc + 32, Vlo + (16 * wave + 8 * half) * 128);                               \
    }                                                                                                         \
  }
#define WP_LOAD_Q()                                                                                           \
  {                                                                                                           \
    tq = token_of(16 * wave + l15);                                                                           \
    const unsigned short* qrow = a.qp + ((long)b * T + (tq >= 0 ? tq : 0)) * a.ldq;                           \
    _Pragma("unroll") for (int ks = 0; ks < 2; ++ks) {                                                        \
      const unsigned short* qq = qrow + 2 * (head * 64 + 32 * ks) + 8 * G;                                    \
      qh[ks] = *reinterpret_cast<const bf16x8*>(qq);                                                          \
      if constexpr (!VF) ql[ks] = *reinterpret_cast<const bf16x8*>(qq + 32);                                  \
    }                                                                                                         \
  }

  {
    const int row = lane >> 2, ch = (lane & 3) ^ ((row >> 2) & 3);
    GLDS16(a.sel + (16 * wave + row) * 32 + ch * 8, Es + 16 * wave * 64);
#pragma unroll 1
    for (int u = wave; u < 16; u += WA_WAVES) {
      const int ks = u >> 3, r0 = 8 * (u & 7);
      const int rrow = r0 + dr;
      const int piece = slot ^ ((rrow & 15) >> 1);
      GLDS16(a.relp + rrow * 128 + 64 * ks + piece * 8, Rs + (ks * 64 + r0) * 128);
    }
  }
  int it = blockIdx.x;
  if (it >= nitems) { asm volatile("s_waitcnt vmcnt(0)" ::: "memory"); return; }
  decode(it);
  bf16x8 qh[2], ql[2];
  int tq;
  WP_ISSUE_K()
  WP_LOAD_Q()

  const int fslot = G ^ ((l15 >> 1) & 7);
  const int frag_hi = l15 * 128 + fslot * 16, frag_lo = l15 * 128 + (fslot ^ 4) * 16;
  const int frag_e = l15 * 64 + ((G ^ ((l15 >> 2) & 3)) << 4);
  constexpr float LOG2E = 1.4426950408889634f;
  const float sc2 = a.scale * LOG2E, rscale = 1.0f / a.scale;
  bool first = true;
  float amax = 0.f;
  int nst_ = 0;

// ... 53 lines not shown
          split2_f16(b1.x, b1.y, hh.z, ll.z);
          split2_f16(b1.z, b1.w, hh.w, ll.w);
        } else {
          split2_f16(b0.x, b0.y, hh.x, ll.x);
          split2_f16(b0.z, b0.w, hh.y, ll.y);
          split2_f16(b1.x, b1.y, hh.z, ll.z);
          split2_f16(b1.z, b1.w, hh.w, ll.w);
        }
        bqh = __builtin_bit_cast(bf16x8, hh);
        bql = __builtin_bit_cast(bf16x8, ll);
      }
    }
    WP_STAMP(2);
    asm volatile("s_waitcnt vmcnt(0)" ::: "memory");
    asm volatile("s_waitcnt lgkmcnt(0)" ::: "memory");
    __syncthreads();
    WP_STAMP(3);
    WP_ISSUE_V()

    f32x4 s[13];
    if (any_live) {
#pragma unroll
      for (int t = 0; t < 13; ++t) {
        const bf16x8 e_ = *reinterpret_cast<const bf16x8*>(Es + 16 * t * 64 + frag_e);
        if constexpr (VF) {
          s[t] = __builtin_amdgcn_mfma_f32_16x16x32_f16(__builtin_bit_cast(f16x8, e_), __builtin_bit_cast(f16x8, bql), (f32x4){0.f, 0.f, 0.f, 0.f}, 0, 0, 0);
          s[t] = __builtin_amdgcn_mfma_f32_16x16x32_f16(__builtin_bit_cast(f16x8, e_), __builtin_bit_cast(f16x8, bqh), s[t], 0, 0, 0);
        } else {
          s[t] = __builtin_amdgcn_mfma_f32_16x16x32_f16(__builtin_bit_cast(f16x8, e_), __builtin_bit_cast(f16x8, bql), (f32x4){0.f, 0.f, 0.f, 0.f}, 0, 0, 0);
          s[t] = __builtin_amdgcn_mfma_f32_16x16x32_f16(__builtin_bit_cast(f16x8, e_), __builtin_bit_cast(f16x8, bqh), s[t], 0, 0, 0);
        }
#pragma unroll
        for (int ks = 0; ks < 2; ++ks) {
          const unsigned char* kb = Ks + (ks * WA_NKEY + 16 * t) * 128;
          const bf16x8 kh_ = *reinterpret_cast<const bf16x8*>(kb + frag_hi);
          if constexpr (VF) {
            s[t] = __builtin_amdgcn_mfma_f32_16x16x32_f16(__builtin_bit_cast(f16x8, kh_), __builtin_bit_cast(f16x8, qh[ks]), s[t], 0, 0, 0);
          } else {
            const bf16x8 kl_ = *reinterpret_cast<const bf16x8*>(kb + frag_lo);
            s[t] = __builtin_amdgcn_mfma_f32_16x16x32_f16(__builtin_bit_cast(f16x8, kl_), __builtin_bit_cast(f16x8, qh[ks]), s[t], 0, 0, 0);
            s[t] = __builtin_amdgcn_mfma_f32_16x16x32_f16(__builtin_bit_cast(f16x8, kh_), __builtin_bit_cast(f16x8, ql[ks]), s[t], 0, 0, 0);
            s[t] = __builtin_amdgcn_mfma_f32_16x16x32_f16(__builtin_bit_cast(f16x8, kh_), __builtin_bit_cast(f16x8, qh[ks]), s[t], 0, 0, 0);
          }
        }
        if (t & 1) __builtin_amdgcn_sched_barrier(0);
      }
    }
    asm volatile("s_waitcnt lgkmcnt(0)" ::: "memory");
    WP_STAMP(4);
    __syncthreads();
    WP_STAMP(5);
    const int it_next = it + gridDim.x;
    const bool has_next = it_next < nitems;
    if (has_next) {
      decode(it_next);
      WP_ISSUE_K()
    }
    float mxs = 0.f;
    if (any_live) {
      int lane_o = lane;
      asm volatile("" : "+v"(lane_o));
      const int G = lane_o >> 4;
      float mx = -INFINITY, mn = INFINITY;
#pragma unroll
      for (int t = 0; t < 13; ++t) {
#if !WP_FOLD
        s[t] *= sc2;
#endif
        if (16 * t + 16 > Nk) {
#pragma unroll
          for (int r = 0; r < 4; ++r) {
            const bool ok = (16 * t + 4 * G + r) < Nk;
            mn = fminf(mn, ok ? s[t][r] : INFINITY);
            s[t][r] = ok ? s[t][r] : -INFINITY;
          }
        } else {
          mn = fminf(fminf(mn, s[t][0]), s[t][1]);
          mn = fminf(fminf(mn, s[t][2]), s[t][3]);
        }
        mx = fmaxf(fmaxf(mx, s[t][0]), s[t][1]);
        mx = fmaxf(fmaxf(mx, s[t][2]), s[t][3]);
      }
      if (live) amax = fmaxf(amax, (WP_FOLD ? sc2 : 1.0f) * fmaxf(fabsf(mx), fabsf(mn)));
      mx = fmaxf(mx, __shfl_xor(mx, 16, 64));
      mx = fmaxf(mx, __shfl_xor(mx, 32, 64));
      mxs = WP_FOLD ? mx * sc2 : mx;
    }
    WP_STAMP(6);
    if (has_next) asm volatile("s_waitcnt vmcnt(4)" ::: "memory");
    else asm volatile("s_waitcnt vmcnt(0)" ::: "memory");
    WP_STAMP(7);
    __syncthreads();
    WP_STAMP(8);
    if (any_live) {
      int lane_o = lane;
      asm volatile("" : "+v"(lane_o));
      const int l15 = lane_o & 15, G = lane_o >> 4;
      f32x4 o[4];
#pragma unroll
      for (int d = 0; d < 4; ++d) o[d] = (f32x4){0.f, 0.f, 0.f, 0.f};
      float psum = 0.f;
#pragma unroll
      for (int g = 0; g < 7; ++g) {
#pragma unroll
        for (int hf = 0; hf < 2; ++hf) {
          if (2 * g + hf < 13) {
#pragma unroll
            for (int r = 0; r < 4; ++r) {
              const float p = WP_FOLD ? __builtin_amdgcn_exp2f(fmaf(s[2 * g + hf][r], sc2, -mxs)) : __builtin_amdgcn_exp2f(s[2 * g + hf][r] - mxs);
              s[2 * g + hf][r] = p;
              psum += p;
            }
          }
        }
        uint4 hh, ll = make_uint4(0u, 0u, 0u, 0u);
        if constexpr (VF) {
          hh.x = pack_f16(s[2 * g][0], s[2 * g][1]);
          hh.y = pack_f16(s[2 * g][2], s[2 * g][3]);
        } else {
          split2_f16(s[2 * g][0], s[2 * g][1], hh.x, ll.x);
          split2_f16(s[2 * g][2], s[2 * g][3], hh.y, ll.y);
        }
// ... 30 lines not shown
          }
        }
        __builtin_amdgcn_sched_barrier(0);
      }
      psum += __shfl_xor(psum, 16, 64);
      psum += __shfl_xor(psum, 32, 64);
      const float inv = 1.0f / psum;
      {
        const long orow = (long)b_cur * T + (tq_cur >= 0 ? tq_cur : 0);
#pragma unroll
        for (int d = 0; d < 4; ++d)
          store_planes8_pair_any<16>(a.op, a.ldo, orow, MMSA_PAD64(a.D), head_cur * 64 + 16 * d + 8 * (G >> 1), make_float4(o[d][0] * inv, o[d][1] * inv, o[d][2] * inv, o[d][3] * inv), a.ofmt, G & 1, tq_cur >= 0);
      }
    }
    WP_STAMP(9);
    ++nst_;
    if (!has_next) break;
    it = it_next;
    WP_LOAD_Q()
  }
  if (a.guard) {
    const float gv = wave_max(amax) * 0.6931471805599453f;
    if (lane == 0 && gv > *reinterpret_cast<volatile float*>(a.guard)) atomicMax(reinterpret_cast<unsigned*>(a.guard), __float_as_uint(gv));
  }
}

extern "C" int mmsa_window_attention_planes(const unsigned short* qkv_planes, long ldq, const unsigned short* bias_planes,
                                            const unsigned short* relpos_planes, const unsigned short* selector,
                                            unsigned short* out_planes, long ldo,
                                            int B, int H, int W, int heads, int head_dim, int window_size, float scale,
                                            int out_fmt, int v_fmt, float* max_abs_logit, hipStream_t stream) {
  MMSA_CHECK_ARG(qkv_planes && bias_planes && relpos_planes && selector && out_planes, "window_attention: null pointer");
  MMSA_CHECK_ARG(out_fmt >= MMSA_FMT_B3 && out_fmt <= MMSA_FMT_F3, "window_attention: bad output plane format %d", out_fmt);
  MMSA_CHECK_ARG(v_fmt == 0 || v_fmt == 2, "window_attention: v_fmt %d (0 = bf16 hi/lo planes; 2 = qkv, bias and rel-pos planes in the h8 format and an fp16 selector: every contraction on the fp16 MFMA)", v_fmt);
  MMSA_CHECK_ARG(B > 0 && H > 0 && W > 0 && heads > 0, "window_attention: bad shape");
  MMSA_CHECK_ARG(head_dim == 64, "window_attention: head_dim %d not supported by this kernel (64)", head_dim);
  MMSA_CHECK_ARG(window_size >= 1 && window_size <= 14, "window_attention: window_size %d not supported (1..14)", window_size);
  const int D = heads * head_dim;
  MMSA_CHECK_ARG(ldq >= 6L * D && (ldq & 63) == 0 && ldo >= (out_fmt == MMSA_FMT_H8C ? 3L : 2L) * D && (ldo & 63) == 0, "window_attention: bad leading dimensions");
  MMSA_CHECK_ARG(((reinterpret_cast<uintptr_t>(qkv_planes) | reinterpret_cast<uintptr_t>(bias_planes) |
                   reinterpret_cast<uintptr_t>(relpos_planes) | reinterpret_cast<uintptr_t>(selector) | reinterpret_cast<uintptr_t>(out_planes)) & 127) == 0,
                 "window_attention: planes must be 128-byte aligned");
  WAttnArgs a;
  a.qp = qkv_planes; a.ldq = ldq; a.bp = bias_planes; a.relp = relpos_planes; a.sel = selector; a.op = out_planes; a.ldo = ldo; a.ofmt = out_fmt;
  a.B = B; a.H = H; a.W = W; a.heads = heads; a.D = D; a.ws = window_size; a.scale = scale;
  a.nWw = cdiv(W, window_size);
  a.guard = max_abs_logit;
#ifdef MMSA_DEBUG_KNOBS
  a.stamps = g_wattn_stamps;
#endif
  a.magic = (unsigned)((65536 + window_size - 1) / window_size);
  for (int j = 0; j < WA_NKV; ++j)
    if ((int)(((unsigned)j * a.magic) >> 16) != j / window_size) {
      mmsa_set_error("window_attention: index arithmetic not exact for window_size %d", window_size);
      return MMSA_ERR_ARG;
    }
  static MmsaPerDevice per_dev_ = {};
  const int num_cus = mmsa_per_device(per_dev_, [] {
    (void)hipFuncSetAttribute((const void*)wattn_persist_kernel<false>, hipFuncAttributeMaxDynamicSharedMemorySize, WP_LDS);
    (void)hipFuncSetAttribute((const void*)wattn_persist_kernel<true>, hipFuncAttributeMaxDynamicSharedMemorySize, WP_LDS);
  });
  const int nWin = cdiv(H, window_size) * a.nWw;
  const int nitems = nWin * heads * B;
  const int nWh_ = cdiv(H, window_size), nWw_ = a.nWw, nHB = heads * B;
  const int n_int = (nWh_ - 1) * (nWw_ - 1) * nHB;
  const int live_h = H - (nWh_ - 1) * window_size, live_w = W - (nWw_ - 1) * window_size;
  const double edge_cost = 0.35 + 0.65 * (0.5 * (live_h + live_w) / window_size);
  auto schedule_cost = [&](int G) {
    double worst = 0.0;
    for (int g = 0; g < G; ++g) {
      double c = 0.0;
      for (int it = g; it < nitems; it += G) c += it < n_int ? 1.0 : edge_cost;
      worst = c > worst ? c : worst;
    }
    return worst;
  };
  const int rounds = cdiv(nitems, num_cus);
  int grid = cdiv(nitems, rounds);
  const int grid_all = nitems < num_cus ? nitems : num_cus;
  if (schedule_cost(grid_all) < schedule_cost(grid) - 1e-9) grid = grid_all;
  if (v_fmt) hipLaunchKernelGGL(wattn_persist_kernel<true>, dim3(grid), dim3(WA_WAVES * 64), WP_LDS, stream, a, nWin, nitems);
  else hipLaunchKernelGGL(wattn_persist_kernel<false>, dim3(grid), dim3(WA_WAVES * 64), WP_LDS, stream, a, nWin, nitems);
  MMSA_CHECK_LAUNCH("window_attention");
  return MMSA_OK;
}
```

multimodal-sam-adapter_amd/mmsa/backbone.py:

```python
import contextlib
import math

import os

import torch
import torch.nn as nn

from . import ops
from .params import CONVNEXT_ARCH, build_tree

_VIT_DEFAULTS = dict(img_size=1024, patch_size=16, in_chans=3, embed_dim=1024, depth=24, mlp_ratio=4.0,
                     qkv_bias=True, use_abs_pos=True, use_rel_pos=True, rel_pos_zero_init=True, window_size=14,
                     global_attn_indexes=[5, 11, 17, 23], pretrained_size=1024, fix=False)


class OperandRangeError(RuntimeError):
    """A forward converted a value beyond the range of an fp16-based operand format (the clamp watch word, include/mmsa.h) and nothing is left to
    re-route: `range_fallback` is off, or the value is a q / k / v (or a qkv bias / rel-pos table entry) beyond +-65504 inside the attention kernels,
    which read fp16-based planes in every mode.  The outputs of that forward are invalid."""


class Workspace:

    def __init__(self, device):
# ... 127 lines not shown
        own = self.state_dict()
        loaded, new = [], {}
        for k, v in sd.items():
            dot = k.find(".")
            for sfx in ("_x", "_y"):
                nk = (k[:dot] + sfx + k[dot:]) if dot != -1 else k + sfx
                full = "spm.twin_conv." + nk
                if full in own:
                    new[full] = v
                    loaded.append(full)
        self.load_state_dict(new, strict=False)
        return loaded

    def invalidate(self):
        self._packed = None
        self._wide_range = False
        self._carry_modes = None
        self._inter_pairs = set()

    def train(self, mode=True):
        if mode:
            raise NotImplementedError("mmsa: the MI355X backbone implements the inference forward path only")
        return super().train(False)

    H8_DEFAULT = ("vit", "inter", "up", "attnv")
    attention_precision = "auto"

    range_fallback = True

    inter_follow_blocks = True

    fp8_weights = False

    def _inter_pair_set(self):
        return set(getattr(self, "_inter_pairs", ()) or ())

    def _interaction_of_block(self, bi):
        for i, idx in enumerate(self.interaction_indexes):
            if idx[0] <= bi <= idx[-1]:
                return i
        return None

    def _wide(self):
        return bool(getattr(self, "_wide_range", False))

    def _pair_fmt(self):
        return ops.FMT_B3 if self._wide() else ops.FMT_F3

    def _h8_sites(self):
        sites = tuple(getattr(self, "h8_sites", self.H8_DEFAULT))
        if self._wide():
            sites = tuple(s_ for s_ in sites if s_ not in ("vit", "inter", "up", "cnx", "cnx2"))
        return sites

    @contextlib.contextmanager
    def chain(self, index):
        base = self._ws
        if base is None:
            raise RuntimeError("mmsa: run one forward() before opening a chain (workspace not created yet)")
        self._ws = _Tagged(base, f"chain{index}_")
        try:
            yield self
        finally:
            self._ws = base

    @torch.no_grad()
# ... 613 lines not shown
            outs.append(f)
        f1, f2, f3, f4 = outs
        return [f1, f2, f3, f4]

    def _stream_planes(self, rows, fmt):
        D = self.cfg["embed_dim"]
        return (self._ws.planes("blk_xp", rows, D, fmt=fmt), self._ws.get("blk_rs", rows, 2 * (D // 64)))

    def _block(self, bp, rel, x, B, Hp, Wp, relg=None, next_fmt=None):
        ws, cfg = self._ws, self.cfg
        D, heads = cfg["embed_dim"], cfg["num_heads"]
        hd = self._hd_pad
        scale = self._hd_true ** -0.5
        Da = heads * hd
        T = Hp * Wp
        folded_w = self._packed["fold_ln"]
        fold = folded_w and B * T >= 128
        fused = bp.get("relp") is not None or relg is not None
        f16 = bp["qkv_bp16"] is not None and self._attn_mode(bp) == "f16"
        vf = bp["qkv"].afmt
        gw = self._packed["attn_guard"][bp["index"]:bp["index"] + 1]
        if fold:
            xp, rs = self._stream_planes(B * T, vf)
            mr = ws.get("blk_mr", B * T, 2)
            ops.rowstats_finalize(rs, B * T, D, 1e-6, mr)
            n = None
        else:
            n = ws.planes("blk_n", B * T, D, fmt=vf)
            if folded_w:
                ops.layernorm(x, self._packed["ln_one"], self._packed["ln_zero"], 1e-6, out_planes=n)
            else:
                ops.layernorm(x, bp["n1w"], bp["n1b"], 1e-6, out_planes=n)
        all16 = fused and f16
        qkv = ws.planes("blk_qkv", B * T, 3 * Da, fmt=ops.FMT_H8 if all16 else ops.FMT_F3)
        if all16:
            bias_p = bp["qkv_bp16"]
        elif f16 and not fused:
            bias_p = bp["qkv_bp"]
            qkv.split = bias_p.split
        else:
            bias_p = bp["qkv_bp_b3"]
        if fold:
            ops.gemm(xp, bp["qkv"], bias=bp["qkv_bf"], out_planes=qkv, row_norm=(mr, bp["qkv_cs"]))
        else:
            ops.gemm(n, bp["qkv"], bias=bp["qkv_bf"] if folded_w else bp["qkv_b"], out_planes=qkv)
        wsz = bp["ws"]
        ao = ws.planes("blk_ao", B * T, Da, fmt=bp["proj"].afmt)
        if bp.get("relp") is not None:
            ops.window_attention(qkv, bias_p, bp["relp16"] if all16 else bp["relp"], ao, B, Hp, Wp, heads, hd, wsz, scale, max_logit=gw)
        elif relg is not None:
            ops.global_attention(qkv, bias_p, relg[1] if all16 else relg[0], ao, B, Hp, Wp, heads, hd, scale, max_logit=gw)
        else:
            kk = 2 * wsz if wsz else Hp + Wp
            rp = ws.get("blk_rp", B * heads * T, kk)
            ops.relpos_bias(qkv, rel[0], rel[1], rp, B, Hp, Wp, heads, hd, wsz)
            ops.attention(qkv, bias_p, rp, ao, B, Hp, Wp, heads, hd, wsz, scale, max_logit=gw)
        vf = bp["lin1"].afmt
        h = ws.planes("blk_h", B * T, bp["lin1"].n, fmt=vf)
        if fold:
            xp, rs = self._stream_planes(B * T, vf)
            ops.gemm(ao, bp["proj"], x, bias=bp["proj_b"], resid=x, out_planes=xp, rowstats_out=rs)
            ops.rowstats_finalize(rs, B * T, D, 1e-6, mr)
            ops.gemm(xp, bp["lin1"], bias=bp["lin1_bf"], act="gelu", out_planes=h, row_norm=(mr, bp["lin1_cs"]))
            if next_fmt is not None:
                xp, rs = self._stream_planes(B * T, next_fmt)
                ops.gemm(h, bp["lin2"], x, bias=bp["lin2_b"], resid=x, out_planes=xp, rowstats_out=rs)
            else:
# ... 477 lines not shown
```

multimodal-sam-adapter_amd/mmsa/lib.py:

```python
import ctypes
import os
from ctypes import c_char_p, c_double, c_float, c_int, c_long, c_void_p, POINTER

_HERE = os.path.dirname(os.path.abspath(__file__))
LIB_PATH = os.environ.get("MMSA_LIB") or os.path.join(_HERE, "libmmsa_hip.so")

if not os.path.exists(LIB_PATH):
    raise RuntimeError(
        f"{LIB_PATH} not found: the MI355X HIP library is required (no CPU/PyTorch fallback exists). "
        "Build it with: python multimodal-sam-adapter_amd/build.py")

import torch

_lib = ctypes.CDLL(LIB_PATH)

P = c_void_p
I = c_int
L = c_long
F = c_float

SIGNATURES = {
    "mmsa_version": [],
    "mmsa_last_error": [],
    "mmsa_debug_poison_lds": [ctypes.c_uint, P],
# ... 25 lines not shown
    "mmsa_gram_tn": [P, L, P, L, L, P, I, I, I, I, P, L, P],
    "mmsa_gram_tn_scratch_bytes": [I, I, I],
    "mmsa_chanattn_build": [P, P, L, P, L, P, P, P, I, I, I, I, P],
    "mmsa_gffm_build": [P, P, P, I, I, I, P],
    "mmsa_gelu_gate": [P, L, P, L, L, I, P],
    "mmsa_pool_hw": [P, L, P, L, I, I, I, I, P],
    "mmsa_ca_apply": [P, L, P, L, P, L, P, L, I, I, I, I, P],
    "mmsa_tail_fuse": [P, L, L, P, L, P, P, P, P, L, I, I, I, I, I, I, P],
    "mmsa_global_attention_planes": [P, L, P, P, P, L, I, I, I, I, I, F, I, I, P, P],
    "mmsa_window_attention_planes": [P, L, P, P, P, P, L, I, I, I, I, I, I, F, I, I, P, P],
    "mmsa_nchw_to_planes": [P, L, P, L, I, I, L, P],
    "mmsa_head_fuse": [P, P, I, I, P, I, I, P, I, I, L, P, P, P, L, P, L, I, I, I, I, I, P],
    "mmsa_tokens_to_nchw": [P, L, P, I, L, I, P],
    "mmsa_bilinear_accum_nchw": [P, L, I, I, I, I, P, I, I, I, I, I, I, P, I, P],
    "mmsa_div_count_nchw": [P, P, I, I, L, P],
    "mmsa_argmax_nchw": [P, P, I, I, L, P],
    "mmsa_crop_batch_nchw": [P, I, I, I, I, P, I, P, I, I, P],
    "mmsa_slide_argmax": [P, I, I, I, I, P, P, I, I, I, I, I, P, P],
    "mmsa_preprocess_nhwc": [P, I, P, I, I, I, I, P, P, P, P, P, P, I, I, P],
    "mmsa_preprocess_crops": [P, I, P, I, I, I, I, P, P, P, P, P, I, I, P, I, P, I, I, P],
    "mmsa_preprocess_resize_nhwc": [P, I, P, I, I, I, I, P, P, P, P, P, P, I, I, I, I, P, P, P, P, I, P],
    "mmsa_preprocess_resize_crops": [P, I, P, I, I, I, I, P, P, P, P, P, I, I, P, I, P, I, I, I, I, P, P, P, P, I, P],
    "mmsa_eval_confusion_u8": [P, P, I, I, I, I, I, P, I, P, P, P, I, P, P],
    "mmsa_slide_argmax_eval": [P, I, I, I, I, P, P, I, I, I, I, I, P, P, I, I, P, P, P, P, I, P, P],
}
_RESTYPES = {"mmsa_last_error": c_char_p, "mmsa_gram_tn_scratch_bytes": c_long}

for _name, _args in SIGNATURES.items():
    _fn = getattr(_lib, _name)
    _fn.argtypes = _args
    _fn.restype = _RESTYPES.get(_name, c_int)


ABI_VERSION = 106
if _lib.mmsa_version() != ABI_VERSION:
    raise RuntimeError(f"{LIB_PATH}: ABI version {_lib.mmsa_version()} but mmsa/lib.py binds version {ABI_VERSION} (include/mmsa.h MMSA_ABI_VERSION): "
                       "rebuild with python multimodal-sam-adapter_amd/build.py")


def last_error() -> str:
    return _lib.mmsa_last_error().decode()


POISON_LDS = os.environ.get("MMSA_DEBUG_POISON_LDS") == "1"


def call(name, *args):
    if POISON_LDS and not name.startswith(("mmsa_event", "mmsa_debug")) and args:
        _lib.mmsa_debug_poison_lds(0x7FC07FC0, args[-1])
    rc = getattr(_lib, name)(*args)
    if rc != 0:
        raise RuntimeError(f"{name} failed (rc={rc}): {last_error()}")


def version() -> int:
    return _lib.mmsa_version()


raw = _lib
```

multimodal-sam-adapter_amd/mmsa/ops.py:

```python
import ctypes

import os

import torch

from . import lib

ACT = {"none": 0, "gelu": 1, "relu": 2, "relu6": 3, "hswish": 4, "sigmoid": 5}

GEMM_PROFILE = None
CLAMP_WATCH = None
GEMM_MAX_GRID = 0
GEMM_FLAVOUR = 0
GEMM_SHAPES = None


def _event():
    ev = ctypes.c_void_p()
    lib.call("mmsa_event_create", ctypes.byref(ev))
    return ev


def collect_gemm_profile(prof):
    flops, ms = 0.0, 0.0
# ... 25 lines not shown

    def __enter__(self):
        global CLAMP_WATCH
        self.keep, CLAMP_WATCH = CLAMP_WATCH, self.word
        return self

    def __exit__(self, *exc):
        global CLAMP_WATCH
        CLAMP_WATCH = self.keep
        return False


def _chk(t, dtype=torch.float32, name="tensor"):
    if t is None:
        return None
    if not t.is_cuda:
        raise RuntimeError(f"mmsa: {name} must live on the GPU (got {t.device}); there is no CPU path")
    if t.dtype != dtype:
        raise RuntimeError(f"mmsa: {name} must be {dtype}, got {t.dtype}")
    if t.device.index != torch.cuda.current_device():
        raise RuntimeError(f"mmsa: {name} lives on {t.device} but the current device is cuda:{torch.cuda.current_device()}; "
                           "call under torch.cuda.device(tensor.device)")
    return t.data_ptr()


def _mat(t, name, dtype=torch.float32):
    if t.dim() != 2 or (t.shape[1] > 1 and t.stride(1) != 1):
        raise RuntimeError(f"mmsa: {name} must be a 2-D view with unit column stride, got shape {tuple(t.shape)} stride {t.stride()}")
    return _chk(t, dtype, name), t.shape[0], t.shape[1], t.stride(0)


FMT_B3, FMT_H8, FMT_H8C, FMT_F3 = 0, 1, 2, 3
FMT_W8 = 4
W8_EMIN, W8_EMAX = -15, 7
E4M3_MAX = 448.0


def _binade(a, lo):
    b = torch.floor(torch.log2(a.clamp_min(2.0 ** (lo - 1)))).clamp_min(lo)
    b = torch.where(a >= torch.exp2(b + 1), b + 1, b)
    return torch.where((b > lo) & (a < torch.exp2(b)), b - 1, b)


def fp8_quantize(w2d):
    w = w2d.detach().to(torch.float64)
    if w.dim() != 2 or not bool(torch.isfinite(w).all()):
        raise ValueError("mmsa.fp8_quantize: a finite 2-D weight is expected")
    amax = w.abs().amax(1) if w.shape[1] else w.new_zeros(w.shape[0])
    lim = E4M3_MAX * 2.0 ** W8_EMAX
    if bool((amax > lim).any()):
        n = int(torch.argmax(amax))
        raise ValueError(f"mmsa.fp8_quantize: row {n} has max |w| = {float(amax[n]):.6g} > {lim:g} = 448 * 2^{W8_EMAX}: not representable as fp8 weights")
    e = torch.ceil(torch.log2(amax.clamp_min(1e-300) / E4M3_MAX)).clamp(W8_EMIN, W8_EMAX)
    e = torch.where(amax > E4M3_MAX * torch.exp2(e), e + 1, e)
    e = torch.where((e > W8_EMIN) & (amax <= E4M3_MAX * torch.exp2(e - 1)), e - 1, e)
    v = w / torch.exp2(e)[:, None]
    a = v.abs()
    step = torch.exp2(_binade(a, -6) - 3)
    q = torch.round(a / step) * step
    b = _binade(q, -6)
    normal = q >= 2.0 ** -6
    code = torch.where(normal, (b + 7) * 8 + (q / torch.exp2(b) * 8 - 8), q * 512.0).to(torch.int32)
    code = code | torch.where((v < 0) & (q > 0), 128, 0)
    return code.to(torch.uint8), e.to(torch.int8)


def fp8_dequantize(codes, exps):
    c = codes.to(torch.int32)
    ex, m = (c >> 3) & 15, (c & 7).double()
    mag = torch.where(ex == 0, m * 2.0 ** -9, (8.0 + m) * torch.exp2(ex.double() - 10.0))
    return (torch.where(c >= 128, -mag, mag) * torch.exp2(exps.double())[:, None]).float()


def w8_planes(w2d):
    n, k = w2d.shape
    if k % 128:
        raise ValueError(f"mmsa.w8_planes: K={k} must be a multiple of 128")
    codes, exps = fp8_quantize(w2d)
    rows = n + -(-((n + 127) // 128 * 128) // k)
    buf = torch.zeros(rows * k, dtype=torch.uint8, device=w2d.device)
    buf[:n * k] = codes.reshape(n, k // 64, 2, 4, 8).permute(0, 1, 3, 2, 4).reshape(-1)
    buf[n * k:n * k + n] = exps.view(torch.uint8)
    return Planes(buf.view(torch.int16).view(rows, k // 2), n, k, k, FMT_W8, True)


def w8_codes(pl):
    n, k = pl.n, pl.kpad
    by = pl.p.contiguous().view(torch.uint8).view(-1)
    return by[:n * k].view(n, k // 64, 4, 2, 8).permute(0, 1, 3, 2, 4).reshape(n, k), by[n * k:n * k + n].view(torch.int8)


class Planes:

    def __init__(self, p, n=None, k=None, kpad=None, fmt=FMT_B3, weight=False, split=0):
        self.p = p
        self.split = split
        if fmt == FMT_H8C and (n is None or kpad is None):
            raise RuntimeError("mmsa.Planes: h8c planes need their row count and padded width (the tensor holds row pairs)")
        self.n = p.shape[0] if n is None else n
        self.kpad = p.shape[1] // 2 if kpad is None else kpad
        self.k = self.kpad if k is None else k
        self.fmt = fmt
        self.weight = weight
        self.gen = None

    @property
    def afmt(self):
        return FMT_H8C if self.fmt == FMT_W8 else self.fmt

    def stamp(self, cell):
        self.gen = (cell, cell[0])
        return self

    def live(self):
        return self.gen is None or self.gen[0][0] == self.gen[1]

    def rows(self, lo, hi=None):
        if self.fmt == FMT_H8C:
            hi = self.n if hi is None else hi
            if lo % 2 or (hi % 2 and hi != self.n):
                raise RuntimeError("mmsa.Planes.rows: h8c planes are stored by row pairs -- slices start and end at even rows")
            return Planes(self.p[lo // 2:(hi + 1) // 2], hi - lo, self.k, self.kpad, self.fmt, self.weight)
        return Planes(self.p[lo:hi], None, self.k, self.kpad, self.fmt, self.weight, self.split)

    def cols(self, lo, hi):
        if lo % 32 or hi % 32 or self.fmt == FMT_H8C:
            raise RuntimeError("mmsa.Planes.cols: column bounds must be multiples of 32 (and the planes bf16 hi/lo or h8 line planes)")
        return Planes(self.p[:, 2 * lo:2 * hi], self.n, hi - lo, hi - lo, self.fmt, self.weight)

    def batch_stride(self, rows):
        if self.fmt == FMT_H8C:
            if rows % 2:
                raise RuntimeError("mmsa.Planes.batch_stride: h8c batches hold an even number of rows")
            return (rows // 2) * self.p.stride(0)
        return rows * self.p.stride(0)

    def mat(self, name):
        ptr, rows, cols, ld = _mat(self.p, name, torch.int16)
        if ptr % 128 or ld % 64:
            raise RuntimeError(f"mmsa: {name} planes must be 128-byte aligned with a row stride that is a multiple of 64")
        if self.fmt == FMT_H8C:
            if ld < 3 * self.kpad or self.kpad % 64:
                raise RuntimeError(f"mmsa: {name}: h8c planes need kpad % 64 == 0 and a pair stride >= 3 * kpad")
            return ptr, self.n, self.kpad, ld
        return ptr, rows, cols // 2, ld


def pad32(k):
    return (k + 31) // 32 * 32


def pad64(k):
    return (k + 63) // 64 * 64


def planes_shape(rows, cols, fmt):
    if fmt == FMT_H8C:
        kp = pad64(cols)
        return (rows + 1) // 2, 3 * kp, kp
    kp = pad32(cols)
    return rows, 2 * kp, kp


def alloc_planes(rows, cols, device, zero=False, fmt=FMT_B3, split=0):
    f = torch.zeros if zero else torch.empty
    if split and (split % 32 or fmt not in (FMT_B3, FMT_F3) or not 0 < split < cols):
        raise RuntimeError(f"mmsa.alloc_planes: split={split} must be a multiple of 32 inside a bf16 hi/lo or f3 matrix of {cols} columns")
    tr, tc, kp = planes_shape(rows, cols, fmt)
    return Planes(f(tr, tc, dtype=torch.int16, device=device), rows, cols, kp, fmt, split=split)


def cp_format(pl):
    return FMT_B3 if pl is None else pl.fmt | ((pl.split // 32) << 8)


def planes_to_float(pl, cols=None):
    r, w = pl.p.shape
    if pl.split:
        lo_part = planes_to_float(Planes(pl.p[:, :2 * pl.split], pl.n, pl.split, pl.split, pl.fmt))
        hi_part = planes_to_float(Planes(pl.p[:, 2 * pl.split:], pl.n, pl.kpad - pl.split, pl.kpad - pl.split, FMT_H8))
        return torch.cat([lo_part, hi_part], 1)[:, :(pl.k if cols is None else cols)]
    if pl.fmt == FMT_W8:
        return fp8_dequantize(*w8_codes(pl))[:, :(pl.k if cols is None else cols)]
    if pl.fmt == FMT_H8C:
        kp = pl.kpad
        by = pl.p[:, :3 * kp].contiguous().view(torch.uint8).view(r, 6 * kp)
        hi = by[:, :4 * kp].contiguous().view(torch.float16).float().reshape(2 * r, kp)
        lo = by[:, 4 * kp:].reshape(r, kp // 64, 2, 4, 2, 8).permute(0, 2, 1, 4, 3, 5)
        lo = lo.contiguous().view(torch.float8_e5m2).float().reshape(2 * r, kp)
        return (hi + lo / (2048.0 * 1.09375))[:pl.n, :(pl.k if cols is None else cols)]
    if pl.fmt == FMT_H8:
        blk = pl.p.contiguous().view(torch.uint8).view(r, w // 64, 128)
        hi = blk[:, :, :64].contiguous().view(torch.float16).float()
        ch = blk[:, :, 64:].reshape(r, w // 64, 4, 2, 8)
        lo = ch[:, :, :, 1 if pl.weight else 0].contiguous().view(torch.float8_e5m2).float().reshape(r, w // 64, 32)
        out = (hi + lo / 2048.0).reshape(r, w // 2)
    elif pl.fmt == FMT_F3:
        v = pl.p.contiguous().view(torch.float16).float().view(r, w // 64, 2, 32)
        out = (v[:, :, 0] + v[:, :, 1]).reshape(r, w // 2)
    else:
        v = (pl.p.to(torch.int32) << 16).view(torch.float32).view(r, w // 64, 2, 32)
        out = (v[:, :, 0] + v[:, :, 1]).reshape(r, w // 2)
    return out[:, :(pl.k if cols is None else cols)]


def split_planes(w2d, kpad=None, out=None, fmt=FMT_B3, weight=False):
    p, n, k, ld = _mat(w2d, "weight")
    if out is None:
        kpad = kpad or (pad64(k) if fmt == FMT_H8C else pad32(k))
        if fmt == FMT_H8C:
            if kpad % 64:
                raise RuntimeError("mmsa.split_planes: h8c planes need kpad % 64 == 0")
            out = Planes(torch.zeros((n + 1) // 2, 3 * kpad, dtype=torch.int16, device=w2d.device), n, k, kpad, fmt, False)
        else:
            out = Planes(torch.empty(n, 2 * kpad, dtype=torch.int16, device=w2d.device), n, k, kpad, fmt, weight)
    kpad = out.kpad
    if out.fmt == FMT_H8C:
        if out.n != n or not out.p.is_contiguous() or out.p.shape[1] != 3 * kpad:
            raise RuntimeError("mmsa.split_planes: dense h8c planes of the source's row count expected")
        kind = 3
    else:
        kind = 0 if out.fmt == FMT_B3 else 4 if out.fmt == FMT_F3 else (2 if out.weight else 1)
    lib.call("mmsa_split_planes", p, ld, n, k, kpad, out.p.data_ptr(), kind, _clamp_ptr(), _stream())
    return out


def gemm(a, w, out=None, bias=None, act="none", alpha=1.0, colscale=None, resid=None, beta=1.0, resid_mod=0,
         batch=1, stride_a=0, stride_w=0, stride_bias=0, stride_r=0, stride_c=0, m=None, pixel_shuffle=None,
         out_planes=None, stride_cp=0, rowstats_out=None, row_norm=None):
    fmt = w.fmt
    if isinstance(a, Planes):
        pap, ma, ka, lda = a.mat("A")
        pa = None
        if ka < w.kpad:
            raise RuntimeError(f"mmsa.gemm: A planes have {ka} columns but the packed weight expects K={w.kpad}")
        if a.fmt != w.afmt or a.weight or (w.fmt == FMT_H8 and not w.weight) or (w.fmt == FMT_H8C and w.weight):
            raise RuntimeError(f"mmsa.gemm: operand formats differ (A fmt {a.fmt}, W fmt {w.fmt} weight={w.weight})")
    elif fmt not in (FMT_B3, FMT_F3):
        raise RuntimeError("mmsa.gemm: h8 weights need A as h8 planes")
    else:
        pa, ma, ka, lda = _mat(a, "A")
        pap = None
        if ka < w.kpad and lda < w.kpad:
            raise RuntimeError(f"mmsa.gemm: A has {ka} columns (ld {lda}) but the packed weight expects K={w.kpad}")
    m = ma if m is None else m
    pc, ldc = None, 0
    if out is not None:
        pc, _, _, ldc = _mat(out, "C")
    pcp, ldcp = None, 0
    if out_planes is not None:
        pcp, _, _, ldcp = out_planes.mat("Cplanes")
    pr, ldr = None, 0
    if resid is not None:
        pr, _, _, ldr = _mat(resid, "resid")
    ps = pixel_shuffle or (0, 0, 0)
    prof = GEMM_PROFILE
    if prof is not None:
        e0, e1 = _event(), _event()
        lib.call("mmsa_event_record", e0, _stream())
    lib.call("mmsa_gemm_split3", pa, pap, lda, stride_a, w.p.data_ptr(), stride_w,
             _chk(bias, name="bias"), stride_bias, _chk(colscale, name="colscale"), pr, ldr, stride_r, resid_mod, beta,
             pc, ldc, stride_c, pcp, ldcp, stride_cp, m, w.n, w.kpad, batch, ACT[act], alpha,
             1 if pixel_shuffle else 0, ps[0], ps[1], ps[2], fmt, cp_format(out_planes), GEMM_MAX_GRID,
             _chk(rowstats_out), _chk(row_norm[0]) if row_norm else None, _chk(row_norm[1]) if row_norm else None, GEMM_FLAVOUR, _clamp_ptr(), _stream())
    if prof is not None:
        lib.call("mmsa_event_record", e1, _stream())
        ob = 3.0 if fmt in (FMT_H8C, FMT_W8) else 4.0
        wb = 1.0 if fmt == FMT_W8 else ob
        pb = 0.0 if out_planes is None else (3.0 if out_planes.fmt == FMT_H8C else 4.0)
        prof.append((2.0 * m * w.n * w.k * batch, e0, e1,
                     batch * (ob * m * w.kpad + wb * w.n * w.kpad + m * w.n * (pb + 4.0 * ((1 if out is not None else 0) + (1 if resid is not None else 0))))))
        if GEMM_SHAPES is not None:
            GEMM_SHAPES.append((m, w.n, w.k, batch, act, resid is not None, ("C" if out is not None else "") + ("P" if out_planes is not None else ""),
                                "planes" if pap is not None else "fp32"))
    return out if out is not None else out_planes


def convnext_mlp_fused(a, w1, w2, b1, b2, gamma, x, m, batch=1, stride_a=0, stride_w1=0, stride_w2=0, stride_x=0):
    pa, _, _, lda = a.mat("A")
    px, _, c, ldx = _mat(x, "x")
    if a.fmt not in (FMT_B3, FMT_F3) or w1.fmt != a.fmt or w2.fmt != a.fmt:
        raise RuntimeError("mmsa.convnext_mlp_fused: bf16 hi/lo or f3 planes expected, the same format for A, W1 and W2")
    prof = GEMM_PROFILE
    if prof is not None:
        e0, e1 = _event(), _event()
        lib.call("mmsa_event_record", e0, _stream())
    lib.call("mmsa_convnext_mlp_fused", pa, lda, stride_a, w1.p.data_ptr(), stride_w1, w2.p.data_ptr(), stride_w2, _chk(b1), _chk(b2),
             _chk(gamma), px, ldx, stride_x, m, c, batch, GEMM_MAX_GRID, a.fmt, _clamp_ptr(), _stream())
    if prof is not None:
        lib.call("mmsa_event_record", e1, _stream())
        prof.append((2.0 * 2.0 * m * c * 4 * c * batch, e0, e1, 4.0 * batch * (m * c * 3 + 2 * 4 * c * c)))
        if GEMM_SHAPES is not None:
            GEMM_SHAPES.append((m, c, 4 * c, batch, "gelu", True, "C", "fused-pair"))
    return x


def convnext_mlp_fused_supported(c):
    return c == 96


def zero_(t):
    if not t.is_contiguous():
# ... 77 lines not shown
        if out is not None:
            po, _, _, ldo = _mat(out, "out")
        pp, ldp = None, 0
        if out_planes is not None:
            pp, _, _, ldp = out_planes.mat("out planes")
        lib.call("mmsa_msda_fused_planes", pvp, ldvp, 1 if lo_bytes else 0, _chk(spatial_shapes, torch.int64), _chk(level_start_index, torch.int64), pr, ldraw,
                 _chk(ref_points), po, ldo, pp, ldp, out_planes.fmt if out_planes is not None else FMT_B3,
                 batch, spatial, heads, d, levels, lq, points, _clamp_ptr(), _stream())
        return out if out is not None else out_planes
    pv, _, _, _ = _mat(value2d, "value")
    po, ldo = None, 0
    if out is not None:
        po, _, _, ldo = _mat(out, "out")
    pp, ldp = None, 0
    if out_planes is not None:
        pp, _, _, ldp = out_planes.mat("out planes")
    lib.call("mmsa_msda_fused", pv, _chk(spatial_shapes, torch.int64), _chk(level_start_index, torch.int64), pr, ldraw,
             _chk(ref_points), po, ldo, pp, ldp, out_planes.fmt if out_planes is not None else FMT_B3,
             batch, spatial, heads, d, levels, lq, points, _clamp_ptr(), _stream())
    return out if out is not None else out_planes


def relpos_bias(qkv, rh, rw, rp, b, h, w, heads, hd, ws):
    if isinstance(qkv, Planes):
        pq, _, _, ldq = qkv.mat("qkv")
        lib.call("mmsa_relpos_bias_planes", pq, ldq, _chk(rh), _chk(rw), _chk(rp), b, h, w, heads, hd, ws, _stream())
    else:
        pq, _, _, ldq = _mat(qkv, "qkv")
        lib.call("mmsa_relpos_bias", pq, ldq, _chk(rh), _chk(rw), _chk(rp), b, h, w, heads, hd, ws, _stream())
    return rp


def _v_fmt(qkv, qkv_bias, d, fused=False, rel=None):
    if qkv.fmt == FMT_H8 or qkv_bias.fmt == FMT_H8 or (rel is not None and rel.fmt == FMT_H8):
        if not (fused and qkv.fmt == FMT_H8 and qkv_bias.fmt == FMT_H8 and rel is not None and rel.fmt == FMT_H8
                and not (qkv.weight or qkv_bias.weight or rel.weight)):
            raise RuntimeError("mmsa attention: h8 planes need the fused rel-pos entry with qkv, bias AND rel-pos planes in the h8 (activation) format")
        return 2
    if qkv.split != qkv_bias.split or qkv.split not in (0, 2 * d) or (fused and qkv.split):
        raise RuntimeError(f"mmsa attention: qkv planes (split {qkv.split}) and bias planes (split {qkv_bias.split}) must both be f3 (fp16 hi/lo) "
                           f"planes, either plain or -- for the entry with a rel-pos prepass -- with the v columns from {2 * d} on as h8 planes")
    if qkv.fmt != FMT_F3 or qkv_bias.fmt != FMT_F3 or (rel is not None and rel.fmt != FMT_F3):
        raise RuntimeError("mmsa attention: the hi/lo operand form of the attention kernels reads f3 planes (fp16 hi/lo pairs: ops.FMT_F3) since round 4 -- "
                           "qkv, bias and rel-pos planes; bf16 hi/lo planes have the same layout and would be misread")
    return 1 if qkv.split else 0


def split_planes_qkv(x2d, d):
    if (2 * d) % 32 or d % 32:
        raise RuntimeError("mmsa.split_planes_qkv: embed dim must be a multiple of 32")
    qk = split_planes(x2d[:, :2 * d].contiguous(), fmt=FMT_F3)
    v = split_planes(x2d[:, 2 * d:].contiguous(), fmt=FMT_H8)
    return Planes(torch.cat([qk.p, v.p], 1).contiguous(), x2d.shape[0], 3 * d, 3 * d, FMT_F3, split=2 * d)


def _guard(g):
    if g is None:
        return None
    if g.dtype != torch.float32 or g.numel() != 1 or not g.is_cuda:
        raise RuntimeError("mmsa attention: max_logit must be a 1-element fp32 device tensor")
    return g.data_ptr()


def attention(qkv, qkv_bias, rp, out, b, h, w, heads, hd, ws, scale, max_logit=None):
    if isinstance(qkv, Planes):
        pq, _, _, ldq = qkv.mat("qkv")
# ... 26 lines not shown
    return split_planes(m, fmt=fmt)


def global_attention(qkv, qkv_bias, relg, out, b, h, w, heads, hd, scale, max_logit=None):
    pq, _, _, ldq = qkv.mat("qkv")
    po, _, _, ldo = out.mat("out")
    lib.call("mmsa_global_attention_planes", pq, ldq, _chk(qkv_bias.p, torch.int16), _chk(relg.p, torch.int16), po, ldo,
             b, h, w, heads, hd, scale, out.fmt, _v_fmt(qkv, qkv_bias, heads * hd, fused=True, rel=relg), _guard(max_logit), _stream())
    return out


_SELECTORS = {}


def window_selector(ws, device, f16=False):
    key = (ws, str(device), f16)
    if key not in _SELECTORS:
        sel = torch.zeros(208, 32, dtype=torch.int16)
        j = torch.arange(min(ws * ws, 208))
        one = 0x3C00
        sel[j, j // ws] = one
        sel[j, 14 + j % ws] = one
        _SELECTORS[key] = sel.to(device)
    return _SELECTORS[key]


def window_attention(qkv, qkv_bias, relp, out, b, h, w, heads, hd, ws, scale, max_logit=None):
    if not 1 <= ws <= 14:
        raise RuntimeError(f"mmsa.window_attention: window_size {ws} not supported (1..14)")
    pq, _, _, ldq = qkv.mat("qkv")
    po, _, _, ldo = out.mat("out")
    vf = _v_fmt(qkv, qkv_bias, heads * hd, fused=True, rel=relp)
    lib.call("mmsa_window_attention_planes", pq, ldq, _chk(qkv_bias.p, torch.int16), _chk(relp.p, torch.int16),
             _chk(window_selector(ws, qkv.p.device, f16=vf == 2), torch.int16), po, ldo, b, h, w, heads, hd, ws, scale, out.fmt,
             vf, _guard(max_logit), _stream())
    return out


def colstats(x, stride_b, b, hw, out, wrow=None, out_is_zero=False):
    px, _, c, ldx = _mat(x, "x")
    lib.call("mmsa_colstats", px, ldx, stride_b, _chk(wrow), b, hw, c, _chk(out, torch.float64), int(out_is_zero), _stream())
    return out


def ffrm_finalize(stats, b, hw, c, mean_w, mean_b, wc, gn_w, gn_b, mean_o, rstd_o, mult_o, scratch):
    lib.call("mmsa_ffrm_finalize", _chk(stats, torch.float64), b, hw, c, mean_w, mean_b, _chk(wc), _chk(gn_w), _chk(gn_b),
             _chk(mean_o), _chk(rstd_o), _chk(mult_o), _chk(scratch), _stream())


def lnhw_apply(x, mean, rstd, mult, w, bias, out, b, hw):
    px, _, c, ldx = _mat(x, "x")
    po, _, _, ldo = _mat(out, "y")
    lib.call("mmsa_lnhw_apply", px, ldx, _chk(mean), _chk(rstd), _chk(mult), _chk(w), _chk(bias), po, ldo, b, hw, c, _stream())
    return out


def dwconv(x, w, bias, out, b, h, wd, k, act="none", xstride_b=None, ystride_b=None, out_planes=None, pstride_b=None,
           imgs_per_group=0, rowstats_out=None):
    px, _, c, ldx = _mat(x, "x")
    po, ldo = None, 0
    if out is not None:
        po, _, _, ldo = _mat(out, "y")
    pp, ldp = None, 0
    if out_planes is not None:
        pp, _, _, ldp = out_planes.mat("y planes")
    xs = h * wd * ldx if xstride_b is None else xstride_b
    ys = h * wd * ldo if ystride_b is None else ystride_b
# ... 98 lines not shown
```

Baseline: 64.29.

## Write qkv GEMM output as fp16-only planes consumed directly by attention

Adds an fp16-only plane format that the h8/h8c/W8 GEMM epilogues can emit for the qkv projection. Because the all-fp16 attention kernels only ever read the hi half, this halves the bytes written and read for the qkv activation. The global and windowed attention kernels gain a template variant that reads these planes with a plain, non-interleaved column index. The cost is more kernel instantiations and a separate epilogue path limited to plain outputs with no activation or residual.

```diff
diff --git a/include/mmsa.h b/include/mmsa.h
--- a/include/mmsa.h
+++ b/include/mmsa.h
@@ -26,7 +26,8 @@
 
 enum { MMSA_DT_F32 = 0, MMSA_DT_F16 = 1, MMSA_DT_F64 = 2 };
 
-enum { MMSA_FMT_B3 = 0, MMSA_FMT_H8 = 1, MMSA_FMT_H8C = 2, MMSA_FMT_F3 = 3, MMSA_FMT_W8 = 4  };
+enum { MMSA_FMT_B3 = 0, MMSA_FMT_H8 = 1, MMSA_FMT_H8C = 2, MMSA_FMT_F3 = 3, MMSA_FMT_W8 = 4 ,
+       MMSA_FMT_F16 = 5  };
 
 int mmsa_ms_deform_attn_forward(const void* value, const int64_t* spatial_shapes, const int64_t* level_start_index,
                                 const void* sampling_loc, const void* attn_weight, void* out, int batch,
diff --git a/include/mmsa_version.h b/include/mmsa_version.h
--- a/include/mmsa_version.h
+++ b/include/mmsa_version.h
@@ -1,4 +1,4 @@
 #ifndef MMSA_VERSION_H
 #define MMSA_VERSION_H
-#define MMSA_ABI_VERSION 106
+#define MMSA_ABI_VERSION 107
 #endif
diff --git a/multimodal-sam-adapter_amd/csrc/attention.hip b/multimodal-sam-adapter_amd/csrc/attention.hip
--- a/multimodal-sam-adapter_amd/csrc/attention.hip
+++ b/multimodal-sam-adapter_amd/csrc/attention.hip
@@ -25,9 +25,11 @@
   float* guard;
 };
 
-template <int HD, bool PL, bool FB, bool REL = false, int VF = 0>
+template <int HD, bool PL, bool FB, bool REL = false, int VF = 0, bool QF = false>
 __global__ __launch_bounds__(256, (FB && HD <= 64) ? 2 : 1) void attn_kernel(AttnArgs a) {
   static_assert(VF == 0 || PL, "the fp16 paths read planes");
+  static_assert(!QF || (VF == 2 && FB), "fp16-only qkv planes feed the all-fp16 form of the global kernel");
+  auto pcol = [](int c) { return QF ? c : ilv(c); };
   static_assert(VF != 2 || REL, "the all-fp16 form exists for the fused rel-pos kernel");
   constexpr int NCH = HD / 8;
   constexpr int KS = HD / 32;
@@ -115,7 +117,7 @@
 #pragma unroll
     for (int ks = 0; ks < KS; ++ks) {
       if constexpr (PL) {
-        const unsigned short* qq = pq_b + qrow + ilv(colq + ks * 32 + 8 * G);
+        const unsigned short* qq = pq_b + qrow + pcol(colq + ks * 32 + 8 * G);
         qh[sub][ks] = *reinterpret_cast<const bf16x8*>(qq);
         if constexpr (VF != 2) ql_[sub][ks] = *reinterpret_cast<const bf16x8*>(qq + 32);
         continue;
@@ -220,8 +222,8 @@
       const unsigned keep_ = tk_ == -2 ? 0u : 0xffffffffu;                                                                     \
       _Pragma("unroll") for (int i = 0; i < NU; ++i) {                                       \
         const int c = squart * (HD / 4) + 8 * i;                                             \
-        const unsigned short* kr_ = rowp_ + ilv(colk + c);                                   \
-        const unsigned short* vr_ = rowp_ + ilv(colv + c);                                   \
+        const unsigned short* kr_ = rowp_ + pcol(colk + c);                                   \
+        const unsigned short* vr_ = rowp_ + pcol(colv + c);                                   \
         rkh[i] = *reinterpret_cast<const uint4*>(kr_);                                       \
         if constexpr (VF != 2) rkl[i] = *reinterpret_cast<const uint4*>(kr_ + 32);           \
         rvh[i] = *reinterpret_cast<const uint4*>(vr_);                                       \
@@ -475,7 +477,7 @@
   MMSA_CHECK_ARG(B > 0 && H > 0 && W > 0 && heads > 0 && window_size >= 0, "attention: bad shape");
   MMSA_CHECK_ARG(head_dim == 64 || head_dim == 32 || head_dim == 96, "attention: head_dim %d not supported (32, 64 or 96; other widths are zero-padded per head by the caller, e.g. ViT-H's 80 -> 96)", head_dim);
   const int D = heads * head_dim;
-  MMSA_CHECK_ARG(a.ldq >= (planes ? 6L : 3L) * D && (a.ldq & 7) == 0 && a.ldo >= (planes ? (a.ofmt == MMSA_FMT_H8C ? 3L * MMSA_PAD64(D) : 2L * D) : 1L * D) && (a.ldo & 3) == 0,
+  MMSA_CHECK_ARG(a.ldq >= ((planes && a.vf != 3) ? 6L : 3L) * D && (a.ldq & 7) == 0 && a.ldo >= (planes ? (a.ofmt == MMSA_FMT_H8C ? 3L * MMSA_PAD64(D) : 2L * D) : 1L * D) && (a.ldo & 3) == 0,
                  "attention: bad leading dimensions");
   a.B = B; a.H = H; a.W = W; a.heads = heads; a.D = D; a.ws = window_size; a.scale = scale;
   int ngroups;
@@ -515,11 +517,12 @@
     if (smem > 64 * 1024) (void)hipFuncSetAttribute((const void*)attn_kernel<HD_, true, FB_, false, 1>, hipFuncAttributeMaxDynamicSharedMemorySize, (int)smem); \
     hipLaunchKernelGGL((attn_kernel<HD_, true, FB_, false, 1>), grid, dim3(256), smem, stream, a);                      \
   } while (0)
-  MMSA_CHECK_ARG(a.vf == 0 || (planes && a.vf == (a.relg ? 2 : 1)), "attention: v_fmt %d (0 = bf16 hi/lo planes; 1 = h8 planes for the v columns, the entry with a rel-pos prepass; 2 = h8 planes throughout, the fused rel-pos entry)", a.vf);
+  MMSA_CHECK_ARG(a.vf == 0 || (planes && (a.vf == (a.relg ? 2 : 1) || (a.relg && a.vf == 3))), "attention: v_fmt %d (0 = bf16 hi/lo planes; 1 = h8 planes for the v columns, the entry with a rel-pos prepass; 2 = h8 planes throughout, the fused rel-pos entry; 3 = that entry with fp16-only qkv planes)", a.vf);
   if (head_dim == 64) {
     if (planes && a.relg) {
       MMSA_CHECK_ARG(fb && H <= 64 && 128 * a.KWs * (int)sizeof(float) <= 2 * 8 * 64 * 16 + 2 * 64 * VSTR, "attention: the fused rel-pos path needs a W = 64, H <= 64 global grid");
-      if (a.vf) hipLaunchKernelGGL((attn_kernel<64, true, true, true, 2>), grid, dim3(256), smem, stream, a);
+      if (a.vf == 3) hipLaunchKernelGGL((attn_kernel<64, true, true, true, 2, true>), grid, dim3(256), smem, stream, a);
+      else if (a.vf) hipLaunchKernelGGL((attn_kernel<64, true, true, true, 2>), grid, dim3(256), smem, stream, a);
       else hipLaunchKernelGGL((attn_kernel<64, true, true, true>), grid, dim3(256), smem, stream, a);
     } else if (planes && a.vf) { if (fb) ATTN_LAUNCH_VF(64, true); else ATTN_LAUNCH_VF(64, false); }
     else if (planes) { if (fb) ATTN_LAUNCH(64, true, true); else ATTN_LAUNCH(64, true, false); }
diff --git a/multimodal-sam-adapter_amd/csrc/common.h b/multimodal-sam-adapter_amd/csrc/common.h
--- a/multimodal-sam-adapter_amd/csrc/common.h
+++ b/multimodal-sam-adapter_amd/csrc/common.h
@@ -160,6 +160,13 @@
   h8_split2<false, COMP>(v.x, v.y, hi.x, lo8, qh8);
   h8_split2<true, COMP>(v.z, v.w, hi.y, lo8, qh8);
 }
+__device__ __forceinline__ unsigned f16_hi2(float a, float b) {
+  a = __builtin_amdgcn_fmed3f(a, -MMSA_H8_MAX, MMSA_H8_MAX);
+  b = __builtin_amdgcn_fmed3f(b, -MMSA_H8_MAX, MMSA_H8_MAX);
+  const mmsa_f32x2 v = {a, b};
+  return __builtin_bit_cast(unsigned, __builtin_convertvector(v, mmsa_h2));
+}
+__device__ __forceinline__ uint2 f16_hi4(const float4 v) { return make_uint2(f16_hi2(v.x, v.y), f16_hi2(v.z, v.w)); }
 __host__ __device__ __forceinline__ int h8_lo_off(int c) { return ((c >> 5) << 7) + 64 + (((c & 31) >> 3) << 4) + (c & 7); }
 
 __device__ __forceinline__ void store_planes4(unsigned short* row, int c, const float4 v, int fmt) {
diff --git a/multimodal-sam-adapter_amd/csrc/gemm_epilogue_regs.inc b/multimodal-sam-adapter_amd/csrc/gemm_epilogue_regs.inc
--- a/multimodal-sam-adapter_amd/csrc/gemm_epilogue_regs.inc
+++ b/multimodal-sam-adapter_amd/csrc/gemm_epilogue_regs.inc
@@ -1,3 +1,7 @@
+#ifndef EPI_F16_PLANES
+#define EPI_F16_PLANES false
+#define EPI_F16_PLANES_DEFAULTED_ 1
+#endif
 #ifndef MMSA_EPI_REGS
 #define MMSA_EPI_REGS 1
 #endif
@@ -77,12 +81,15 @@
               prow = pb + (row0 & 1) * cp_kpad + nb_ + hcol;
               plo = reinterpret_cast<unsigned char*>(pb + 2 * cp_kpad) + (row0 & 1) * 64 + ((nb_ >> 6) << 7) + schunk;
               pstep = 8 * a.ldcp;
+            } else if constexpr (kCPF == MMSA_FMT_F16) {
+              prow = Cp + (long)row0 * a.ldcp + nb_ + hcol;
+              pstep = 16 * a.ldcp;
             } else if constexpr (kCPF >= 0) {
               prow = Cp + (long)row0 * a.ldcp + ((nb_ >> 5) << 6) + hcol;
               pstep = 16 * a.ldcp;
             }
             unsigned long long cwm_ = 0ull;
-            constexpr bool kWatch = MMSA_CLAMP_WATCH && MMSA_CW_REGS && (kCPF == MMSA_FMT_H8C || kCPF == MMSA_FMT_H8 || kCPF == MMSA_FMT_F3);
+            constexpr bool kWatch = MMSA_CLAMP_WATCH && MMSA_CW_REGS && (kCPF == MMSA_FMT_H8C || kCPF == MMSA_FMT_H8 || kCPF == MMSA_FMT_F3 || kCPF == MMSA_FMT_F16);
             constexpr float kLimit = (kCPF == MMSA_FMT_F3) ? MMSA_F3_MAX : MMSA_H8_MAX;
             float* rsb = nullptr;
             if constexpr (kRS) rsb = a.rs_out + (((long)bz * a.M + row0) * a.rs_strips + (nb_ >> 6)) * 2;
@@ -119,6 +126,7 @@
                 if constexpr (kWatch) cwm_ |= __builtin_amdgcn_ballot_w64(fmaxf(fmaxf(fabsf(o.x), fabsf(o.y)), fmaxf(fabsf(o.z), fabsf(o.w))) > kLimit);
                 if constexpr (kCPF == MMSA_FMT_H8C) h8_split4<true>(o, H[ni], L8[ni], Q8[ni]);
                 else if constexpr (kCPF == MMSA_FMT_H8) h8_split4<false>(o, H[ni], L8[ni], Q8[ni]);
+                else if constexpr (kCPF == MMSA_FMT_F16) H[ni] = f16_hi4(o);
                 else if constexpr (kCPF == MMSA_FMT_F3) f3_split4(o, H[ni], Lp[ni]);
                 else if constexpr (kCPF == MMSA_FMT_B3) split4(o, H[ni], Lp[ni]);
               }
@@ -129,7 +137,7 @@
                   swap16_(H[2 * p].x, H[2 * p + 1].x);
                   swap16_(H[2 * p].y, H[2 * p + 1].y);
                   const uint4 hv = make_uint4(H[2 * p].x, H[2 * p].y, H[2 * p + 1].x, H[2 * p + 1].y);
-                  if constexpr (kCPF == MMSA_FMT_H8C) {
+                  if constexpr (kCPF == MMSA_FMT_H8C || kCPF == MMSA_FMT_F16) {
                     EPI_ST16(pr + 32 * p, hv)
                   } else {
                     EPI_ST16(pr + 64 * p, hv)
@@ -236,6 +244,9 @@
   { epi_regs_(std::integral_constant<bool, C_>{}, std::integral_constant<bool, R_>{}, std::integral_constant<int, F_>{},               \
               std::integral_constant<bool, S_>{}, std::integral_constant<bool, N_>{}, std::integral_constant<bool, CS_>{}); regs_done = true; }
 #define EPI_REGS_RUN(C_, R_, F_, S_, N_) { if (!scaled_) EPI_REGS_RUN1(C_, R_, F_, S_, N_, false) }
+          if constexpr (EPI_F16_PLANES) {
+            if (!C && !resid && !rso_ && cpf_ == MMSA_FMT_F16) { if (rn_) EPI_REGS_RUN(false, false, MMSA_FMT_F16, false, true) else EPI_REGS_RUN(false, false, MMSA_FMT_F16, false, false) }
+          } else
           if (!C && !resid && !rso_) {
             if (cpf_ == MMSA_FMT_H8C) { if (rn_) EPI_REGS_RUN(false, false, MMSA_FMT_H8C, false, true) else EPI_REGS_RUN(false, false, MMSA_FMT_H8C, false, false) }
             else if (cpf_ == MMSA_FMT_H8) { if (rn_) EPI_REGS_RUN(false, false, MMSA_FMT_H8, false, true) else EPI_REGS_RUN(false, false, MMSA_FMT_H8, false, false) }
diff --git a/multimodal-sam-adapter_amd/csrc/gemm_h8c.hip b/multimodal-sam-adapter_amd/csrc/gemm_h8c.hip
--- a/multimodal-sam-adapter_amd/csrc/gemm_h8c.hip
+++ b/multimodal-sam-adapter_amd/csrc/gemm_h8c.hip
@@ -16,8 +16,9 @@
 #define EPI_STAMP(i_)
 #define EPI_STAMP_WAIT()
 #endif
-template <bool GEN, int ACT>
+template <bool GEN, int ACT, bool F16P = false>
 __global__ __launch_bounds__(512, 1) void gemm_h8c_kernel(GemmV2Args a) {
+  static_assert(!F16P || (!GEN && ACT == ACT_NONE), "fp16-only planes: plain output, no activation");
   constexpr bool PP = true;
   constexpr bool EPI_UNROLL = ACT >= 0;
   constexpr int V2_BM = 256;
@@ -190,6 +191,7 @@
 #endif
       EPI_STAMP(0)
 #define EPI_STAGING_BASE (smem + (((j - 1) & 1) ? 2 * HC_H_UNIT + HC_L_UNIT : 2 * HC_H_UNIT))
+#define EPI_F16_PLANES F16P
 #include "gemm_v2_epilogue.inc"
       EPI_STAMP(7)
 #ifdef HC_EPI_STAMP
@@ -214,9 +216,11 @@
 #define HC_ATTR(GEN_, ACT_) (void)hipFuncSetAttribute((const void*)gemm_h8c_kernel<GEN_, ACT_>, hipFuncAttributeMaxDynamicSharedMemorySize, HC_LDS_TOTAL);
     V2_EPI_TABLE(HC_ATTR)
 #undef HC_ATTR
+    (void)hipFuncSetAttribute((const void*)gemm_h8c_kernel<false, ACT_NONE, true>, hipFuncAttributeMaxDynamicSharedMemorySize, HC_LDS_TOTAL);
   });
 #define HC_LAUNCH(GEN_, ACT_) if (v2_epi_serves(gen, act, GEN_, ACT_)) hipLaunchKernelGGL((gemm_h8c_kernel<GEN_, ACT_>), dim3(grid), dim3(512), HC_LDS_TOTAL, stream, a);
-  V2_EPI_TABLE(HC_LAUNCH)
+  if (MMSA_CP_BASE(a.cp_fmt) == MMSA_FMT_F16) hipLaunchKernelGGL((gemm_h8c_kernel<false, ACT_NONE, true>), dim3(grid), dim3(512), HC_LDS_TOTAL, stream, a);
+  else { V2_EPI_TABLE(HC_LAUNCH) }
 #undef HC_LAUNCH
   MMSA_CHECK_LAUNCH("gemm_split3(h8c)");
   return MMSA_OK;
diff --git a/multimodal-sam-adapter_amd/csrc/gemm_h8c_w8.hip b/multimodal-sam-adapter_amd/csrc/gemm_h8c_w8.hip
--- a/multimodal-sam-adapter_amd/csrc/gemm_h8c_w8.hip
+++ b/multimodal-sam-adapter_amd/csrc/gemm_h8c_w8.hip
@@ -14,8 +14,9 @@
   return make_uint2(__builtin_bit_cast(unsigned, lo), __builtin_bit_cast(unsigned, hi));
 }
 
-template <bool GEN, int ACT>
+template <bool GEN, int ACT, bool F16P = false>
 __global__ __launch_bounds__(512, 1) void gemm_h8c_w8_kernel(GemmV2Args a) {
+  static_assert(!F16P || (!GEN && ACT == ACT_NONE), "fp16-only planes: plain output, no activation");
   constexpr bool PP = true;
   constexpr bool EPI_UNROLL = ACT >= 0;
   constexpr int V2_BM = 256;
@@ -225,6 +226,7 @@
     if (!grp) H8C_BAR()
     if (V2_DBG(a) == 2) H8C_NO_EPILOGUE() else {
 #define EPI_STAGING_BASE (smem + ((((j - 1) >> 1) & 1) ? HW_LDS_L(1) - 16384 : HW_LDS_L(0)))
+#define EPI_F16_PLANES F16P
 #include "gemm_v2_epilogue.inc"
     }
     asm volatile("s_waitcnt lgkmcnt(0)" ::: "memory");
@@ -239,9 +241,11 @@
 #define HW_ATTR(GEN_, ACT_) (void)hipFuncSetAttribute((const void*)gemm_h8c_w8_kernel<GEN_, ACT_>, hipFuncAttributeMaxDynamicSharedMemorySize, HW_LDS_TOTAL);
     V2_EPI_TABLE(HW_ATTR)
 #undef HW_ATTR
+    (void)hipFuncSetAttribute((const void*)gemm_h8c_w8_kernel<false, ACT_NONE, true>, hipFuncAttributeMaxDynamicSharedMemorySize, HW_LDS_TOTAL);
   });
 #define HW_LAUNCH(GEN_, ACT_) if (v2_epi_serves(gen, act, GEN_, ACT_)) hipLaunchKernelGGL((gemm_h8c_w8_kernel<GEN_, ACT_>), dim3(grid), dim3(512), HW_LDS_TOTAL, stream, a);
-  V2_EPI_TABLE(HW_LAUNCH)
+  if (MMSA_CP_BASE(a.cp_fmt) == MMSA_FMT_F16) hipLaunchKernelGGL((gemm_h8c_w8_kernel<false, ACT_NONE, true>), dim3(grid), dim3(512), HW_LDS_TOTAL, stream, a);
+  else { V2_EPI_TABLE(HW_LAUNCH) }
 #undef HW_LAUNCH
   MMSA_CHECK_LAUNCH("gemm_split3(h8c x w8)");
   return MMSA_OK;
diff --git a/multimodal-sam-adapter_amd/csrc/gemm_split3.hip b/multimodal-sam-adapter_amd/csrc/gemm_split3.hip
--- a/multimodal-sam-adapter_amd/csrc/gemm_split3.hip
+++ b/multimodal-sam-adapter_amd/csrc/gemm_split3.hip
@@ -309,7 +309,11 @@
   MMSA_CHECK_ARG(!(rs_out && rn_mr), "gemm_split3: a GEMM either writes row statistics or normalises by them");
   const bool extras = rs_out || rn_mr;
   MMSA_CHECK_ARG(!extras || (ap && M >= 128), "gemm_split3: row statistics / row normalisation need activation planes and M >= 128");
-  MMSA_CHECK_ARG(fmt >= MMSA_FMT_B3 && fmt <= MMSA_FMT_W8 && cp_fmt >= 0 && MMSA_CP_BASE(cp_fmt) >= MMSA_FMT_B3 && MMSA_CP_BASE(cp_fmt) <= MMSA_FMT_F3, "gemm_split3: bad plane format %d / %d", fmt, cp_fmt);
+  MMSA_CHECK_ARG(fmt >= MMSA_FMT_B3 && fmt <= MMSA_FMT_W8 && cp_fmt >= 0 && ((MMSA_CP_BASE(cp_fmt) >= MMSA_FMT_B3 && MMSA_CP_BASE(cp_fmt) <= MMSA_FMT_F3) || MMSA_CP_BASE(cp_fmt) == MMSA_FMT_F16), "gemm_split3: bad plane format %d / %d", fmt, cp_fmt);
+  const bool cp_f16 = MMSA_CP_BASE(cp_fmt) == MMSA_FMT_F16;
+  MMSA_CHECK_ARG(!cp_f16 || (Cp && !C && !resid && !rs_out && ap && out_mode == 0 && resid_mod <= 0 && act == ACT_NONE && MMSA_CP_SPLIT(cp_fmt) == 0 &&
+                             (fmt == MMSA_FMT_H8 || fmt == MMSA_FMT_H8C || fmt == MMSA_FMT_W8) && flavour != 4),
+                 "gemm_split3: fp16-only output planes (cp_fmt %d) are written by the h8 / h8c / W8 kernels as a plain planes-only output without activation, residual or row statistics", cp_fmt);
   MMSA_CHECK_ARG(MMSA_CP_SPLIT(cp_fmt) == 0 || (out_mode == 0 && MMSA_CP_SPLIT(cp_fmt) < N && MMSA_CP_BASE(cp_fmt) != MMSA_FMT_H8C), "gemm_split3: the output-format split %d needs a plain [M, N] bf16 hi/lo planes output with N=%d beyond it", MMSA_CP_SPLIT(cp_fmt), N);
   MMSA_CHECK_ARG(fmt == MMSA_FMT_B3 || fmt == MMSA_FMT_F3 || (ap && K % 64 == 0), "gemm_split3: h8 / h8c operands need A planes and K %% 64 == 0 (K=%d)", K);
   MMSA_CHECK_ARG(fmt != MMSA_FMT_F3 || ap || !Cp, "gemm_split3: f3 weights with an fp32 A write fp32 outputs only");
@@ -337,7 +341,7 @@
     MMSA_CHECK_ARG((!C || ldc >= ps_C) && (!Cp || ldcp >= (cp_h8c ? 3L * MMSA_PAD64(ps_C) : 2L * ps_C)), "gemm_split3: ldc < C");
   } else {
     MMSA_CHECK_ARG(out_mode == 0, "gemm_split3: bad out_mode %d", out_mode);
-    MMSA_CHECK_ARG((!C || ldc >= N) && (!Cp || ldcp >= (cp_h8c ? 3L * MMSA_PAD64(N) : 2L * ((N + 31) / 32 * 32))), "gemm_split3: ldc=%ld < N=%d", ldc, N);
+    MMSA_CHECK_ARG((!C || ldc >= N) && (!Cp || ldcp >= (cp_h8c ? 3L * MMSA_PAD64(N) : cp_f16 ? (long)MMSA_PAD64(N) : 2L * ((N + 31) / 32 * 32))), "gemm_split3: ldc=%ld < N=%d", ldc, N);
   }
   GemmArgs a;
   a.A = A; a.Ap = Ap; a.lda = lda; a.strideA = strideA;
diff --git a/multimodal-sam-adapter_amd/csrc/gemm_v2.hip b/multimodal-sam-adapter_amd/csrc/gemm_v2.hip
--- a/multimodal-sam-adapter_amd/csrc/gemm_v2.hip
+++ b/multimodal-sam-adapter_amd/csrc/gemm_v2.hip
@@ -1,7 +1,8 @@
 #include "common.h"
 #include "gemm_v2_shared.h"
-template <bool GEN, int ACT, bool PP, int NW, int FMT>
+template <bool GEN, int ACT, bool PP, int NW, int FMT, bool F16P = false>
 __global__ __launch_bounds__(NW * 64, NW == 4 ? 2 : 1) void gemm_v2_kernel(GemmV2Args a) {
+  static_assert(!F16P || (!GEN && ACT == ACT_NONE && FMT == MMSA_FMT_H8), "fp16-only planes: plain output of the h8 flavour, no activation");
   static_assert(NW == 8 || (NW == 4 && !PP), "4-wave workgroups run the in-phase main loop");
   static_assert(FMT == MMSA_FMT_B3 || (PP && NW == 8), "the h8 and f3 operand formats run on the ping-pong kernel");
   constexpr bool EPI_UNROLL = ACT >= 0;
@@ -430,6 +431,7 @@
 
     if (V2_DBG(a) == 2 || V2_DBG(a) == 5 || V2_DBG(a) >= 64) { tile += G; continue; }
 #define EPI_STAGING_BASE (smem + st_cur * V2_STAGE)
+#define EPI_F16_PLANES F16P
 #include "gemm_v2_epilogue.inc"
     if constexpr (PP) {
       asm volatile("s_waitcnt lgkmcnt(0)" ::: "memory");
@@ -505,6 +507,7 @@
   (void)hipFuncSetAttribute((const void*)gemm_v2_kernel<GEN_, ACT_, false, 4, MMSA_FMT_B3>, hipFuncAttributeMaxDynamicSharedMemorySize, V2_LDS_BYTES(4));
     V2_EPI_TABLE(V2_ATTR)
 #undef V2_ATTR
+    (void)hipFuncSetAttribute((const void*)gemm_v2_kernel<false, ACT_NONE, true, 8, MMSA_FMT_H8, true>, hipFuncAttributeMaxDynamicSharedMemorySize, V2_LDS_BYTES(8));
   });
   const int cus = (max_grid > 0 && max_grid < num_cus) ? max_grid : num_cus;
   const bool h8c4 = flavour == 4 && h8c && !w8 && out_mode == 0 && resid_mod <= 0 && act == ACT_NONE && M >= 128;
@@ -564,7 +567,11 @@
     else if (pp) hipLaunchKernelGGL((gemm_v2_kernel<GEN_, ACT_, true, 8, MMSA_FMT_B3>), dim3(grid), dim3(512), V2_LDS_BYTES(8), stream, a);     \
     else hipLaunchKernelGGL((gemm_v2_kernel<GEN_, ACT_, false, 8, MMSA_FMT_B3>), dim3(grid), dim3(512), V2_LDS_BYTES(8), stream, a);            \
   }
-  V2_EPI_TABLE(V2_LAUNCH)
+  if (MMSA_CP_BASE(cp_fmt) == MMSA_FMT_F16) {
+    hipLaunchKernelGGL((gemm_v2_kernel<false, ACT_NONE, true, 8, MMSA_FMT_H8, true>), dim3(grid), dim3(512), V2_LDS_BYTES(8), stream, a);
+  } else {
+    V2_EPI_TABLE(V2_LAUNCH)
+  }
 #undef V2_LAUNCH
   MMSA_CHECK_LAUNCH("gemm_split3(v2)");
   return MMSA_OK;
diff --git a/multimodal-sam-adapter_amd/csrc/gemm_v2_epilogue.inc b/multimodal-sam-adapter_amd/csrc/gemm_v2_epilogue.inc
--- a/multimodal-sam-adapter_amd/csrc/gemm_v2_epilogue.inc
+++ b/multimodal-sam-adapter_amd/csrc/gemm_v2_epilogue.inc
@@ -30,8 +30,9 @@
       const bool cp_h8c = cp_base == MMSA_FMT_H8C;
       const int cp_kpad = MMSA_PAD64((GEN && a.out_mode == 1) ? a.ps_C : a.N);
 #include "gemm_epilogue_regs.inc"
+      const bool cp_f16 = EPI_F16_PLANES && cp_base == MMSA_FMT_F16;
       if (!regs_done) {
-      const float cw_lim_ = cp_split ? MMSA_H8_MAX : mmsa_clamp_limit(cp_base);
+      const float cw_lim_ = (cp_split || cp_f16) ? MMSA_H8_MAX : mmsa_clamp_limit(cp_base);
       auto cp_stage4 = [&](unsigned short* srow_, int c_, const float4 o_, int col_) {
 #if MMSA_CW_LEG
         { float m_ = 0.f; clamp_see(m_, o_); clamp_report(a.clamp_max, m_, cw_lim_); }
@@ -41,6 +42,8 @@
           h8_split4<true>(o_, hi_, lo8_, qh8_);
           *reinterpret_cast<uint2*>(srow_ + c_) = hi_;
           *reinterpret_cast<unsigned*>(reinterpret_cast<unsigned char*>(srow_) + 128 + h8c_lo_off(c_)) = lo8_;
+        } else if (cp_f16) {
+          *reinterpret_cast<uint2*>(srow_ + c_) = f16_hi4(o_);
         } else {
           store_planes4(srow_, c_, o_, cp_split ? MMSA_CP_AT(a.cp_fmt, col_) : cp_base);
         }
@@ -51,6 +54,8 @@
           const int l_ = lane & 15, ch_ = (dcol__ >> 6) << 7;
           if (l_ < 8) *reinterpret_cast<uint4*>(reinterpret_cast<unsigned char*>(r_.hi) + ch_ + 16 * l_) = pk_;
           else if (l_ < 12) *reinterpret_cast<uint4*>(r_.lo + ch_ + 16 * (l_ - 8)) = pk_;
+        } else if (cp_f16) {
+          if ((lane & 15) < 8) *reinterpret_cast<uint4*>(Cp + drow__ * a.ldcp + (dcol__ & ~63) + 8 * (lane & 15)) = pk_;
         } else {
           *reinterpret_cast<uint4*>(Cp + drow__ * a.ldcp + ilv(dcol__ & ~63) + 8 * (lane & 15)) = pk_;
         }
@@ -60,6 +65,7 @@
         clamp_report(a.clamp_max, fabsf(x_), cw_lim_);
 #endif
         if (cp_h8c) h8c_store1(h8c_row(Cp, a.ldcp, drow__, cp_kpad), dcol__, x_);
+        else if (cp_f16) Cp[drow__ * a.ldcp + dcol__] = (unsigned short)(f16_hi2(x_, 0.f) & 0xFFFFu);
         else store_planes1(Cp + drow__ * a.ldcp, dcol__, x_, MMSA_CP_AT(a.cp_fmt, dcol__));
       };
       const int rl0 = lane >> 4;
@@ -313,6 +319,10 @@
     }
     }
 #undef EPI_STAGING_BASE
+#ifdef EPI_F16_PLANES_DEFAULTED_
+#undef EPI_F16_PLANES_DEFAULTED_
+#endif
+#undef EPI_F16_PLANES
 #ifdef EPI_STAMP_DEFAULTED_
 #undef EPI_STAMP_DEFAULTED_
 #undef EPI_STAMP
diff --git a/multimodal-sam-adapter_amd/csrc/wattn.hip b/multimodal-sam-adapter_amd/csrc/wattn.hip
--- a/multimodal-sam-adapter_amd/csrc/wattn.hip
+++ b/multimodal-sam-adapter_amd/csrc/wattn.hip
@@ -50,8 +50,9 @@
 #define WP_R_BYTES (2 * 64 * 128)
 #define WP_LDS (WA_K_BYTES + 2 * WP_V_BYTES + WA_E_BYTES + WP_R_BYTES + WA_WAVES * WA_B_BYTES)
 
-template <bool VF>
+template <bool VF, bool QF = false>
 __global__ __launch_bounds__(WA_WAVES * 64) void wattn_persist_kernel(WAttnArgs a, int nWin, int nitems) {
+  static_assert(!QF || VF, "fp16-only qkv planes feed the all-fp16 form");
   extern __shared__ __attribute__((aligned(16))) unsigned char smem[];
   unsigned char* Ks = smem;
   unsigned char* Vhi = smem + WA_K_BYTES;
@@ -102,8 +103,13 @@
       const int t_ = token_of(key);                                                                           \
       const unsigned short* row = t_ >= 0 ? pq_b_ + (long)t_ * a.ldq : a.bp;                                  \
       const int piece = slot ^ ((key & 15) >> 1);                                                             \
-      GLDS16(row + 2 * colk_ + piece * 8, Ks + (16 * wave + 8 * half) * 128);                                 \
-      GLDS16(row + 2 * (colk_ + 32) + piece * 8, Ks + (WA_NKEY + 16 * wave + 8 * half) * 128);                \
+      if constexpr (QF) {    \
+        const int off_ = t_ >= 0 ? colk_ + piece * 8 : 2 * colk_ + (piece >> 2) * 64 + (piece & 3) * 8;       \
+        GLDS16(row + off_, Ks + (16 * wave + 8 * half) * 128);                                                \
+      } else {                                                                                                \
+        GLDS16(row + 2 * colk_ + piece * 8, Ks + (16 * wave + 8 * half) * 128);                               \
+        GLDS16(row + 2 * (colk_ + 32) + piece * 8, Ks + (WA_NKEY + 16 * wave + 8 * half) * 128);              \
+      }                                                                                                       \
     }                                                                                                         \
   }
 #define WP_ISSUE_V()                                                                                          \
@@ -118,7 +124,7 @@
       const int t_ = token_of(key);                                                                           \
       const unsigned short* row = t_ >= 0 ? pq_b_ + (long)t_ * a.ldq : a.bp;                                  \
       const int c = slot ^ (((key >> 1) & 3) << 1);                                                           \
-      const unsigned short* vsrc = row + 2 * (colv_ + 32 * (c >> 2)) + (c & 3) * 8;                           \
+      const unsigned short* vsrc = (QF && t_ >= 0) ? row + colv_ + c * 8 : row + 2 * (colv_ + 32 * (c >> 2)) + (c & 3) * 8; \
       GLDS16(vsrc, Vhi + (16 * wave + 8 * half) * 128);                                                       \
       if constexpr (!VF) GLDS16(vsrc + 32, Vlo + (16 * wave + 8 * half) * 128);                               \
     }                                                                                                         \
@@ -128,7 +134,7 @@
     tq = token_of(16 * wave + l15);                                                                           \
     const unsigned short* qrow = a.qp + ((long)b * T + (tq >= 0 ? tq : 0)) * a.ldq;                           \
     _Pragma("unroll") for (int ks = 0; ks < 2; ++ks) {                                                        \
-      const unsigned short* qq = qrow + 2 * (head * 64 + 32 * ks) + 8 * G;                                    \
+      const unsigned short* qq = qrow + (QF ? 1 : 2) * (head * 64 + 32 * ks) + 8 * G;                         \
       qh[ks] = *reinterpret_cast<const bf16x8*>(qq);                                                          \
       if constexpr (!VF) ql[ks] = *reinterpret_cast<const bf16x8*>(qq + 32);                                  \
     }                                                                                                         \
@@ -248,8 +254,8 @@
         }
 #pragma unroll
         for (int ks = 0; ks < 2; ++ks) {
-          const unsigned char* kb = Ks + (ks * WA_NKEY + 16 * t) * 128;
-          const bf16x8 kh_ = *reinterpret_cast<const bf16x8*>(kb + frag_hi);
+          const unsigned char* kb = Ks + ((QF ? 0 : ks * WA_NKEY) + 16 * t) * 128;
+          const bf16x8 kh_ = *reinterpret_cast<const bf16x8*>(kb + ((QF && ks) ? frag_lo : frag_hi));
           if constexpr (VF) {
             s[t] = __builtin_amdgcn_mfma_f32_16x16x32_f16(__builtin_bit_cast(f16x8, kh_), __builtin_bit_cast(f16x8, qh[ks]), s[t], 0, 0, 0);
           } else {
@@ -303,7 +309,7 @@
       mxs = WP_FOLD ? mx * sc2 : mx;
     }
     WP_STAMP(6);
-    if (has_next) asm volatile("s_waitcnt vmcnt(4)" ::: "memory");
+    if (has_next) { if constexpr (QF) asm volatile("s_waitcnt vmcnt(2)" ::: "memory"); else asm volatile("s_waitcnt vmcnt(4)" ::: "memory"); }
     else asm volatile("s_waitcnt vmcnt(0)" ::: "memory");
     WP_STAMP(7);
     __syncthreads();
@@ -400,12 +406,12 @@
                                             int out_fmt, int v_fmt, float* max_abs_logit, hipStream_t stream) {
   MMSA_CHECK_ARG(qkv_planes && bias_planes && relpos_planes && selector && out_planes, "window_attention: null pointer");
   MMSA_CHECK_ARG(out_fmt >= MMSA_FMT_B3 && out_fmt <= MMSA_FMT_F3, "window_attention: bad output plane format %d", out_fmt);
-  MMSA_CHECK_ARG(v_fmt == 0 || v_fmt == 2, "window_attention: v_fmt %d (0 = bf16 hi/lo planes; 2 = qkv, bias and rel-pos planes in the h8 format and an fp16 selector: every contraction on the fp16 MFMA)", v_fmt);
+  MMSA_CHECK_ARG(v_fmt == 0 || v_fmt == 2 || v_fmt == 3, "window_attention: v_fmt %d (0 = bf16 hi/lo planes; 2 = qkv, bias and rel-pos planes in the h8 format and an fp16 selector: every contraction on the fp16 MFMA; 3 = the same with the qkv planes as fp16-only planes)", v_fmt);
   MMSA_CHECK_ARG(B > 0 && H > 0 && W > 0 && heads > 0, "window_attention: bad shape");
   MMSA_CHECK_ARG(head_dim == 64, "window_attention: head_dim %d not supported by this kernel (64)", head_dim);
   MMSA_CHECK_ARG(window_size >= 1 && window_size <= 14, "window_attention: window_size %d not supported (1..14)", window_size);
   const int D = heads * head_dim;
-  MMSA_CHECK_ARG(ldq >= 6L * D && (ldq & 63) == 0 && ldo >= (out_fmt == MMSA_FMT_H8C ? 3L : 2L) * D && (ldo & 63) == 0, "window_attention: bad leading dimensions");
+  MMSA_CHECK_ARG(ldq >= (v_fmt == 3 ? 3L : 6L) * D && (ldq & 63) == 0 && ldo >= (out_fmt == MMSA_FMT_H8C ? 3L : 2L) * D && (ldo & 63) == 0, "window_attention: bad leading dimensions");
   MMSA_CHECK_ARG(((reinterpret_cast<uintptr_t>(qkv_planes) | reinterpret_cast<uintptr_t>(bias_planes) |
                    reinterpret_cast<uintptr_t>(relpos_planes) | reinterpret_cast<uintptr_t>(selector) | reinterpret_cast<uintptr_t>(out_planes)) & 127) == 0,
                  "window_attention: planes must be 128-byte aligned");
@@ -427,6 +433,7 @@
   const int num_cus = mmsa_per_device(per_dev_, [] {
     (void)hipFuncSetAttribute((const void*)wattn_persist_kernel<false>, hipFuncAttributeMaxDynamicSharedMemorySize, WP_LDS);
     (void)hipFuncSetAttribute((const void*)wattn_persist_kernel<true>, hipFuncAttributeMaxDynamicSharedMemorySize, WP_LDS);
+    (void)hipFuncSetAttribute((const void*)wattn_persist_kernel<true, true>, hipFuncAttributeMaxDynamicSharedMemorySize, WP_LDS);
   });
   const int nWin = cdiv(H, window_size) * a.nWw;
   const int nitems = nWin * heads * B;
@@ -447,7 +454,8 @@
   int grid = cdiv(nitems, rounds);
   const int grid_all = nitems < num_cus ? nitems : num_cus;
   if (schedule_cost(grid_all) < schedule_cost(grid) - 1e-9) grid = grid_all;
-  if (v_fmt) hipLaunchKernelGGL(wattn_persist_kernel<true>, dim3(grid), dim3(WA_WAVES * 64), WP_LDS, stream, a, nWin, nitems);
+  if (v_fmt == 3) hipLaunchKernelGGL((wattn_persist_kernel<true, true>), dim3(grid), dim3(WA_WAVES * 64), WP_LDS, stream, a, nWin, nitems);
+  else if (v_fmt) hipLaunchKernelGGL(wattn_persist_kernel<true>, dim3(grid), dim3(WA_WAVES * 64), WP_LDS, stream, a, nWin, nitems);
   else hipLaunchKernelGGL(wattn_persist_kernel<false>, dim3(grid), dim3(WA_WAVES * 64), WP_LDS, stream, a, nWin, nitems);
   MMSA_CHECK_LAUNCH("window_attention");
   return MMSA_OK;
diff --git a/multimodal-sam-adapter_amd/mmsa/backbone.py b/multimodal-sam-adapter_amd/mmsa/backbone.py
--- a/multimodal-sam-adapter_amd/mmsa/backbone.py
+++ b/multimodal-sam-adapter_amd/mmsa/backbone.py
@@ -183,6 +183,8 @@
 
     fp8_weights = False
 
+    qkv_f16_planes = True
+
     def _inter_pair_set(self):
         return set(getattr(self, "_inter_pairs", ()) or ())
 
@@ -862,7 +864,9 @@
             else:
                 ops.layernorm(x, bp["n1w"], bp["n1b"], 1e-6, out_planes=n)
         all16 = fused and f16
-        qkv = ws.planes("blk_qkv", B * T, 3 * Da, fmt=ops.FMT_H8 if all16 else ops.FMT_F3)
+        f16p = (all16 and bool(getattr(self, "qkv_f16_planes", True)) and B * T >= 128 and ops.GEMM_FLAVOUR != 4
+                and bp["qkv"].fmt in (ops.FMT_H8, ops.FMT_H8C, ops.FMT_W8))
+        qkv = ws.planes("blk_qkv", B * T, 3 * Da, fmt=ops.FMT_F16 if f16p else ops.FMT_H8 if all16 else ops.FMT_F3)
         if all16:
             bias_p = bp["qkv_bp16"]
         elif f16 and not fused:
diff --git a/multimodal-sam-adapter_amd/mmsa/lib.py b/multimodal-sam-adapter_amd/mmsa/lib.py
--- a/multimodal-sam-adapter_amd/mmsa/lib.py
+++ b/multimodal-sam-adapter_amd/mmsa/lib.py
@@ -81,7 +81,7 @@
     _fn.restype = _RESTYPES.get(_name, c_int)
 
 
-ABI_VERSION = 106
+ABI_VERSION = 107
 if _lib.mmsa_version() != ABI_VERSION:
     raise RuntimeError(f"{LIB_PATH}: ABI version {_lib.mmsa_version()} but mmsa/lib.py binds version {ABI_VERSION} (include/mmsa.h MMSA_ABI_VERSION): "
                        "rebuild with python multimodal-sam-adapter_amd/build.py")
diff --git a/multimodal-sam-adapter_amd/mmsa/ops.py b/multimodal-sam-adapter_amd/mmsa/ops.py
--- a/multimodal-sam-adapter_amd/mmsa/ops.py
+++ b/multimodal-sam-adapter_amd/mmsa/ops.py
@@ -81,6 +81,7 @@
 
 FMT_B3, FMT_H8, FMT_H8C, FMT_F3 = 0, 1, 2, 3
 FMT_W8 = 4
+FMT_F16 = 5
 W8_EMIN, W8_EMAX = -15, 7
 E4M3_MAX = 448.0
 
@@ -147,7 +148,7 @@
         if fmt == FMT_H8C and (n is None or kpad is None):
             raise RuntimeError("mmsa.Planes: h8c planes need their row count and padded width (the tensor holds row pairs)")
         self.n = p.shape[0] if n is None else n
-        self.kpad = p.shape[1] // 2 if kpad is None else kpad
+        self.kpad = (p.shape[1] if fmt == FMT_F16 else p.shape[1] // 2) if kpad is None else kpad
         self.k = self.kpad if k is None else k
         self.fmt = fmt
         self.weight = weight
@@ -173,7 +174,7 @@
         return Planes(self.p[lo:hi], None, self.k, self.kpad, self.fmt, self.weight, self.split)
 
     def cols(self, lo, hi):
-        if lo % 32 or hi % 32 or self.fmt == FMT_H8C:
+        if lo % 32 or hi % 32 or self.fmt in (FMT_H8C, FMT_F16):
             raise RuntimeError("mmsa.Planes.cols: column bounds must be multiples of 32 (and the planes bf16 hi/lo or h8 line planes)")
         return Planes(self.p[:, 2 * lo:2 * hi], self.n, hi - lo, hi - lo, self.fmt, self.weight)
 
@@ -192,6 +193,10 @@
             if ld < 3 * self.kpad or self.kpad % 64:
                 raise RuntimeError(f"mmsa: {name}: h8c planes need kpad % 64 == 0 and a pair stride >= 3 * kpad")
             return ptr, self.n, self.kpad, ld
+        if self.fmt == FMT_F16:
+            if self.kpad % 64 or ld < self.kpad:
+                raise RuntimeError(f"mmsa: {name}: fp16-only planes need kpad % 64 == 0 and a row stride >= kpad")
+            return ptr, rows, self.kpad, ld
         return ptr, rows, cols // 2, ld
 
 
@@ -207,6 +212,9 @@
     if fmt == FMT_H8C:
         kp = pad64(cols)
         return (rows + 1) // 2, 3 * kp, kp
+    if fmt == FMT_F16:
+        kp = pad64(cols)
+        return rows, kp, kp
     kp = pad32(cols)
     return rows, 2 * kp, kp
 
@@ -238,6 +246,8 @@
         lo = by[:, 4 * kp:].reshape(r, kp // 64, 2, 4, 2, 8).permute(0, 2, 1, 4, 3, 5)
         lo = lo.contiguous().view(torch.float8_e5m2).float().reshape(2 * r, kp)
         return (hi + lo / (2048.0 * 1.09375))[:pl.n, :(pl.k if cols is None else cols)]
+    if pl.fmt == FMT_F16:
+        return pl.p.contiguous().view(torch.float16).float()[:, :(pl.k if cols is None else cols)]
     if pl.fmt == FMT_H8:
         blk = pl.p.contiguous().view(torch.uint8).view(r, w // 64, 128)
         hi = blk[:, :, :64].contiguous().view(torch.float16).float()
@@ -264,6 +274,8 @@
         else:
             out = Planes(torch.empty(n, 2 * kpad, dtype=torch.int16, device=w2d.device), n, k, kpad, fmt, weight)
     kpad = out.kpad
+    if out.fmt in (FMT_W8, FMT_F16):
+        raise RuntimeError("mmsa.split_planes: W8 weights are packed by w8_planes; fp16-only planes are written by the qkv GEMM only")
     if out.fmt == FMT_H8C:
         if out.n != n or not out.p.is_contiguous() or out.p.shape[1] != 3 * kpad:
             raise RuntimeError("mmsa.split_planes: dense h8c planes of the source's row count expected")
@@ -316,7 +328,7 @@
         lib.call("mmsa_event_record", e1, _stream())
         ob = 3.0 if fmt in (FMT_H8C, FMT_W8) else 4.0
         wb = 1.0 if fmt == FMT_W8 else ob
-        pb = 0.0 if out_planes is None else (3.0 if out_planes.fmt == FMT_H8C else 4.0)
+        pb = 0.0 if out_planes is None else (3.0 if out_planes.fmt == FMT_H8C else 2.0 if out_planes.fmt == FMT_F16 else 4.0)
         prof.append((2.0 * m * w.n * w.k * batch, e0, e1,
                      batch * (ob * m * w.kpad + wb * w.n * w.kpad + m * w.n * (pb + 4.0 * ((1 if out is not None else 0) + (1 if resid is not None else 0))))))
         if GEMM_SHAPES is not None:
@@ -460,6 +472,10 @@
 
 
 def _v_fmt(qkv, qkv_bias, d, fused=False, rel=None):
+    if qkv.fmt == FMT_F16:
+        if not (fused and qkv_bias.fmt == FMT_H8 and rel is not None and rel.fmt == FMT_H8 and not (qkv.weight or qkv_bias.weight or rel.weight or qkv.split)):
+            raise RuntimeError("mmsa attention: fp16-only qkv planes need the fused rel-pos entry with bias AND rel-pos planes in the h8 (activation) format")
+        return 3
     if qkv.fmt == FMT_H8 or qkv_bias.fmt == FMT_H8 or (rel is not None and rel.fmt == FMT_H8):
         if not (fused and qkv.fmt == FMT_H8 and qkv_bias.fmt == FMT_H8 and rel is not None and rel.fmt == FMT_H8
                 and not (qkv.weight or qkv_bias.weight or rel.weight)):
@@ -552,7 +568,7 @@
     po, _, _, ldo = out.mat("out")
     vf = _v_fmt(qkv, qkv_bias, heads * hd, fused=True, rel=relp)
     lib.call("mmsa_window_attention_planes", pq, ldq, _chk(qkv_bias.p, torch.int16), _chk(relp.p, torch.int16),
-             _chk(window_selector(ws, qkv.p.device, f16=vf == 2), torch.int16), po, ldo, b, h, w, heads, hd, ws, scale, out.fmt,
+             _chk(window_selector(ws, qkv.p.device, f16=vf in (2, 3)), torch.int16), po, ldo, b, h, w, heads, hd, ws, scale, out.fmt,
              vf, _guard(max_logit), _stream())
     return out
 
```

Result: no change. 64.69 (median of 2 runs) (+0.6%).
